# aiforvision/OCTA-autosegmentation

Hardware: AMD Instinct MI355X
Metric: synthetic OCTA samples/sec (graph + 304x304 image + 1216x1216 label triples) (higher is better)
Workload: dtype f64

## Files before the change

include/octa_hip.h:

```cpp
#ifndef OCTA_HIP_H
#define OCTA_HIP_H

#include <stddef.h>
#include <stdint.h>

#ifdef __cplusplus
extern "C" {
#endif

typedef struct octa_ctx octa_ctx;


int octa_abi_version(void);

const char *octa_last_error(void);

int octa_ctx_create(int device, octa_ctx **out);
void octa_ctx_destroy(octa_ctx *ctx);

size_t octa_ctx_scratch_bytes(const octa_ctx *ctx);

int octa_rasterize_2d(octa_ctx *ctx, int B, const double *d_edges, const int64_t *h_edge_off,
                      const uint8_t *d_keep, int no_pixels_x, int no_pixels_y, int mip_axis,
                      double min_radius, double max_radius, uint8_t *d_out, void *stream);
// ... 140 lines not shown
int octa_menten_floater(octa_ctx *ctx, const double *d_img, const int *d_pts, const int *d_npts, const int *d_dilations, const double *d_weights,
                        int radius, int B, int P, int N, unsigned char *d_mask, int *d_dist, double *d_tmp, double *d_out, void *stream);
int octa_menten_motion(octa_ctx *ctx, const void *d_in, void *d_out, int elem_size, const int *d_table, const void *d_white, int n_white,
                       int unit_elems, int B, int H, int W, void *stream);

int octa_noise_model(octa_ctx *ctx, const float *d_img, const float *d_background, const float *d_grids, int B, int H, int W, int gh, int gw,
                     uint64_t seed, uint32_t sample_offset, double lambda_delta, double lambda_speckle, double lambda_gamma,
                     const float *d_delta_in, const float *d_n_in, float *d_out, float *d_maps, float *d_fields, void *stream);
void octa_philox4x32_10(const uint32_t *counter4, const uint32_t *key2, uint32_t *out4);

int octa_noise_model_backward(octa_ctx *ctx, const float *d_dout, const float *d_img, const float *d_background, const float *d_grids, int B, int H,
                              int W, int gh, int gw, uint64_t seed, uint32_t sample_offset, double lambda_delta, double lambda_speckle,
                              double lambda_gamma, const float *d_delta_in, const float *d_n_in, float *d_dgrids, float *d_dmaps, float *d_out,
                              float *d_maps, float *d_logodds, float *d_bgrad, void *stream);

int octa_conv3x3_c1_fwd(octa_ctx *ctx, const void *d_x, const float *d_w, void *d_y, int N, int H, int W, int Cout, double *d_stat, int nslot,
                        void *stream);
int octa_conv3x3_c1_wgrad(octa_ctx *ctx, const void *d_x, const void *d_dy, float *d_dw, int N, int H, int W, int Cout, void *stream);

int octa_dice_bce_fwd(octa_ctx *ctx, const void *d_logits, int dtype, const float *d_y, int B, int64_t n, double *d_sums, void *stream);
int octa_dice_bce_finish(octa_ctx *ctx, const double *d_sums, int B, int64_t n, double smooth_nr, double smooth_dr, float *d_loss, void *stream);
int octa_dice_bce_bwd(octa_ctx *ctx, const void *d_logits, int dtype, const float *d_y, int B, int64_t n, const double *d_sums,
                      const float *d_grad_out, float smooth_nr, float smooth_dr, void *d_dlogits, void *stream);

int octa_thinconv_expand(octa_ctx *ctx, const void *d_s, const void *d_w, const void *d_bias, void *d_out, int N, int Hs, int Ws, int C, int K,
                         int pad, int flip, float slope, void *stream);
int octa_thinconv_squeeze(octa_ctx *ctx, const void *d_a, const void *d_w, const void *d_bias, void *d_out, int N, int Ha, int Wa, int C, int K,
                          int pad, int flip, void *stream);
long long octa_thinconv_wgrad_scratch_floats(int N, int Ha, int C, int K);
int octa_lrelu_bwd_bf16(octa_ctx *ctx, const void *d_y, const void *d_dy, void *d_out, int64_t n, float slope, void *stream);
int octa_thinconv_wgrad(octa_ctx *ctx, const void *d_a, const void *d_s, void *d_scratch, void *d_g, void *d_asum, int N, int Ha, int Wa, int Hs,
                        int Ws, int C, int K, int pad, int flip, void *stream);

int octa_reflect_pad_fwd(octa_ctx *ctx, const void *d_in, void *d_out, int dtype, int B, int H, int W, int C, int pad, void *stream);
int octa_reflect_pad_bwd(octa_ctx *ctx, const void *d_in, void *d_out, int dtype, int B, int H, int W, int C, int pad, void *stream);
int octa_blur_down_fwd(octa_ctx *ctx, const void *d_in, void *d_out, int dtype, int B, int H, int W, int C, void *stream);
int octa_blur_down_bwd(octa_ctx *ctx, const void *d_in, void *d_out, int dtype, int B, int H, int W, int C, void *stream);
int octa_blur_up_fwd(octa_ctx *ctx, const void *d_in, void *d_out, int dtype, int B, int H, int W, int C, void *stream);
int octa_blur_up_bwd(octa_ctx *ctx, const void *d_in, void *d_out, int dtype, int B, int H, int W, int C, void *stream);

int octa_remove_small_objects(octa_ctx *ctx, const uint8_t *d_in, int B, int H, int W, int min_size, int connectivity,
                              uint8_t on_value, uint8_t *d_out, void *stream);

int octa_skeletonize(octa_ctx *ctx, const uint8_t *d_in, int B, int H, int W, uint8_t *d_out, int *passes, void *stream);


size_t octa_fft2_c2c_f64_workspace_bytes(int b, int h, int w);

int octa_fft2_c2c_f64(const void *d_in, void *d_out, int b, int h, int w, int inverse, void *d_ws, void *stream);

size_t octa_oof_workspace_bytes(int b, int h, int w);

int octa_oof_2d(const float *d_in, double *d_out, int b, int h, int w, void *d_ws, void *stream);

int octa_oof_2d_response(const float *d_in, double *d_out, int b, int h, int w, void *d_ws, void *stream);


size_t octa_frangi_workspace_bytes(int b, int h, int w, int n_scales);

int octa_frangi_2d(const float *d_in, double *d_out, int b, int h, int w, int n_scales, const int *radii, const double *weights, float in_scale,
                   double beta, double gamma, int black_ridges, void *d_ws, void *stream);

int octa_frangi_hessian(const float *d_in, float *d_hrr, float *d_hrc, float *d_hcc, int b, int h, int w, int radius, const double *weights,
                        float in_scale, int black_ridges, void *d_ws, void *stream);

int octa_frangi_eigenvalues(const float *d_in, float *d_l1, float *d_l2, float *d_gamma, int b, int h, int w, int radius, const double *weights,
                            float in_scale, int black_ridges, void *d_ws, void *stream);

typedef struct octa_sim octa_sim;

typedef struct {
    double param_scale, d, r;
    double faz_radius_mean, faz_radius_std;
    double rotation_radius;
    double faz_center[2];
    double size[3];
    int n_trees;
    int walls[4];
    int n_modes;
    double modes[8][13];
    int forest_type;
    double nerve_center[2];
    double nerve_radius;
    const uint8_t *geometry;
    int geometry_shape[3];
    int n_source_walls;
    int source_walls[6];
} octa_sim_config;

#define OCTA_BIF_MAX_ATTS 256
typedef struct {
    int sample, n;
    double pos[3];
    double r, kappa, d;
    double atts[OCTA_BIF_MAX_ATTS * 3];
} octa_bif_request;

typedef void (*octa_bif_fn)(int n_req, const octa_bif_request *reqs, double *out6, void *user);

int octa_bif_native_init(const char *blas_path, int n_kappa, const double *kappas, const double *cs, const double *sn,
                         octa_bif_fn fallback, void *fallback_user);
void octa_bif_native(int n_req, const octa_bif_request *reqs, double *out6, void *user);
int octa_bif_native_counts(int64_t *h_out2);

int octa_sim_create(octa_ctx *ctx, const octa_sim_config *cfg, int B, octa_sim **out);
int octa_sim_create_ex(octa_ctx *ctx, const octa_sim_config *cfg, int B, int build, octa_sim **out);
void octa_sim_destroy(octa_sim *sim);

long long octa_sim_launch_count(void);
int octa_order_wait_launch(octa_ctx *ctx, long long ticket, int timeout_us, int settle_us, int *d_out3, void *stream);

int octa_sim_run(octa_sim *sim, const uint32_t *h_np_seeds, const uint64_t *h_py_seeds, octa_bif_fn bif, void *user,
                 void *stream);

int octa_sim_run_states(octa_sim *sim, const double *h_faz_radius, const double *h_stumps, const uint32_t *h_np_states,
                        const uint32_t *h_py_states, octa_bif_fn bif, void *user, void *stream);
int octa_sim_np_state(octa_sim *sim, int sample, uint32_t *h_state625);

int octa_sim_edge_offsets(octa_sim *sim, int64_t *h_edge_off, int64_t *h_n_art);

int octa_sim_export_edges(octa_sim *sim, double *h_edges);

int octa_sim_export_edges_device(octa_sim *sim, double *d_edges, void *stream);

int octa_sim_trace(octa_sim *sim, int32_t *h_trace);

int octa_sim_stats(octa_sim *sim, int64_t *h_stats);

int octa_sim_kd_paths(octa_sim *sim, int64_t *h_paths);

int octa_sim_assign_paths(octa_sim *sim, int64_t *h_paths);

int octa_sim_spans(octa_sim *sim, int64_t *h_spans);

int octa_sim_timing(octa_sim *sim, double *h_out8);

int octa_sim_service_stats(octa_sim *sim, double *h_out5);

int octa_sim_geometry(int num_cus, int *h_out4);

int octa_sim_is_large(const octa_sim *sim);

int octa_sim_fields(octa_sim *sim, int sample, double *h_oxy, int64_t cap_oxy, int64_t *n_oxy, double *h_co2,
                    int64_t cap_co2, int64_t *n_co2);

int octa_sim_kat_kd_order(octa_ctx *ctx, const double *h_pts, int64_t n, const uint8_t *h_need, int32_t *h_indices);

int octa_sim_kat_kd_order_signflag(octa_ctx *ctx, const double *h_pts, int64_t n, const uint8_t *h_need, int32_t need_bits, int32_t *h_indices);

int octa_sim_kat_sample(octa_ctx *ctx, const double *h_cand, int64_t n_cand, const double *h_npos, const double *h_nrad, int64_t n_art,
                        double *h_oxy, int64_t n_oxy, int64_t cap_oxy, double eps_n, double eps_k, double eps_s, const double *h_cst8,
                        int64_t *h_n_out);

#ifdef __cplusplus
}
#endif
#endif
```

octa_autosegmentation_amd/_native.py:

```python
import contextlib
import ctypes
import os
import random as _random
import threading

import numpy as np

HERE = os.path.dirname(os.path.abspath(__file__))
LIB_PATH = os.environ.get("OCTA_HIP_LIB") or os.path.join(HERE, "liboctahip.so")

_lib = None
_ctxs = {}
_lock = threading.Lock()

c_void_p, c_int, c_double, c_size_t = ctypes.c_void_p, ctypes.c_int, ctypes.c_double, ctypes.c_size_t


def _struct(name, ints, ptrs):
    fields = [("struct_size", ctypes.c_uint32)] + [(k, c_int) for k in ints.split()] + [("slope", ctypes.c_float)] + [(k, c_void_p) for k in ptrs.split()]
    return type(name, (ctypes.Structure,), {"_fields_": fields})


Conv3x3Args = _struct("Conv3x3Args", "N H W Cin Cout stride in_dilation tap_mask out_scale out_off_y out_off_x C1 CY1 nslot",
                      "d_x d_x2 d_w d_y d_y2 d_scale1 d_shift1 d_scale2 d_shift2 d_stat_partials d_stat_slots d_residual")
Conv3x3WgradArgs = _struct("Conv3x3WgradArgs", "N H W Cin Cout stride tap_mask C1 out_mode", "d_x d_x2 d_dy d_dw d_scale1 d_shift1 d_scale2 d_shift2")
WGRAD_TAP_MAJOR, WGRAD_PARAM_ADD, WGRAD_PARAM_SET = 0, 1, 2

SIGNATURES = {
    "octa_abi_version": (c_int, []),
    "octa_last_error": (ctypes.c_char_p, []),
    "octa_ctx_create": (c_int, [c_int, ctypes.POINTER(c_void_p)]),
    "octa_ctx_destroy": (None, [c_void_p]),
    "octa_ctx_scratch_bytes": (c_size_t, [c_void_p]),
    "octa_rasterize_2d": (c_int, [c_void_p, c_int, c_void_p, c_void_p, c_void_p, c_int, c_int, c_int, c_double,
                                  c_double, c_void_p, c_void_p]),
    "octa_rasterize_2d_plan": (c_int, [c_void_p, c_int, c_void_p, c_void_p, c_void_p, c_int, c_int, c_int, c_double, c_double, c_void_p]),
    "octa_rasterize_2d_draw": (c_int, [c_void_p, c_void_p, c_void_p]),
    "octa_raster_prof": (c_int, [c_void_p, c_void_p]),
    "octa_fs_dither": (c_int, [c_void_p, c_int, c_void_p, c_int, c_int, c_void_p, c_void_p]),
    "octa_voxel_padded_dims": (c_int, [c_void_p, c_void_p]),
    "octa_voxelize_3d": (c_int, [c_void_p, c_int, c_void_p, c_void_p, c_void_p, c_void_p, c_double, c_double, c_int, c_void_p, c_void_p]),
    "octa_edges_read_back": (c_int, [c_void_p, c_void_p, c_void_p, ctypes.c_int64, c_void_p, c_void_p]),
    "octa_max_u8": (c_int, [c_void_p, c_void_p, c_void_p, c_void_p, c_size_t, c_void_p]),
    "octa_bif_native_init": (c_int, [ctypes.c_char_p, c_int, c_void_p, c_void_p, c_void_p, c_void_p, c_void_p]),
    "octa_bif_native": (None, [c_int, c_void_p, c_void_p, c_void_p]),
    "octa_bif_native_counts": (c_int, [c_void_p]),
    "octa_instnorm_lrelu_fwd": (c_int, [c_void_p] * 7 + [c_int, c_int, ctypes.c_int64, c_int, ctypes.c_float, ctypes.c_float, c_void_p]),
    "octa_instnorm_lrelu_bwd": (c_int, [c_void_p] * 10 + [c_int, c_int, ctypes.c_int64, c_int, ctypes.c_float, c_void_p]),
    "octa_csv_bytes_bound": (ctypes.c_int64, [ctypes.c_int64]),
    "octa_csv_format_edges": (ctypes.c_int64, [c_void_p, ctypes.c_int64, c_void_p, ctypes.c_int64]),
    "octa_csv_write_file": (c_int, [ctypes.c_char_p, c_void_p, ctypes.c_int64]),
    "octa_csv_count_rows": (ctypes.c_int64, [c_void_p, ctypes.c_int64]),
    "octa_csv_parse_edges": (ctypes.c_int64, [c_void_p, ctypes.c_int64, c_void_p, ctypes.c_int64]),
    "octa_py_random_advance": (c_int, [c_void_p, ctypes.c_int64]),
    "octa_png_write_gray8": (c_int, [ctypes.c_char_p, c_void_p, c_int, c_int, c_int]),
    "octa_png_write_bits": (c_int, [ctypes.c_char_p, c_void_p, c_int, c_int, c_int]),
    "octa_write_sample_files": (c_int, [ctypes.c_int64, c_void_p, c_void_p, c_void_p, c_void_p, c_void_p, c_int, c_int, c_void_p, c_int, c_int, c_int,
                                        ctypes.c_char_p, ctypes.c_int64, c_int, c_int]),
    "octa_pack_bits": (c_int, [c_void_p, c_void_p, c_void_p, ctypes.c_int64, c_int, c_void_p]),
    "octa_background_noise": (c_int, [c_void_p, c_void_p, c_void_p, c_void_p, ctypes.c_int64, c_void_p, c_void_p, c_void_p]),
    "octa_speckle_brightness": (c_int, [c_void_p, c_void_p, c_void_p, c_void_p, c_int, c_int, c_int, c_void_p, c_void_p, c_void_p]),
    "octa_menten_vessel_noise": (c_int, [c_void_p, c_void_p, c_int, c_void_p, c_void_p, c_void_p, c_int, c_double, c_double, c_int, c_int, c_int, c_void_p, c_void_p, c_void_p]),
    "octa_menten_floater_mask": (c_int, [c_void_p, c_void_p, c_void_p, c_void_p, c_int, c_int, c_int, c_void_p, c_void_p, c_void_p]),
    "octa_menten_floater": (c_int, [c_void_p, c_void_p, c_void_p, c_void_p, c_void_p, c_void_p, c_int, c_int, c_int, c_int, c_void_p, c_void_p, c_void_p, c_void_p, c_void_p]),
    "octa_menten_motion": (c_int, [c_void_p, c_void_p, c_void_p, c_int, c_void_p, c_void_p, c_int, c_int, c_int, c_int, c_int, c_void_p]),
    "octa_noise_model": (c_int, [c_void_p, c_void_p, c_void_p, c_void_p, c_int, c_int, c_int, c_int, c_int, ctypes.c_uint64, ctypes.c_uint32, c_double, c_double, c_double,
                                 c_void_p, c_void_p, c_void_p, c_void_p, c_void_p, c_void_p]),
    "octa_noise_model_backward": (c_int, [c_void_p, c_void_p, c_void_p, c_void_p, c_void_p, c_int, c_int, c_int, c_int, c_int, ctypes.c_uint64, ctypes.c_uint32,
                                          c_double, c_double, c_double, c_void_p, c_void_p, c_void_p, c_void_p, c_void_p, c_void_p, c_void_p, c_void_p, c_void_p]),
    "octa_philox4x32_10": (None, [c_void_p, c_void_p, c_void_p]),
    "octa_sim_create": (c_int, [c_void_p, c_void_p, c_int, ctypes.POINTER(c_void_p)]),
    "octa_sim_create_ex": (c_int, [c_void_p, c_void_p, c_int, c_int, ctypes.POINTER(c_void_p)]),
    "octa_sim_destroy": (None, [c_void_p]),
    "octa_sim_run": (c_int, [c_void_p, c_void_p, c_void_p, c_void_p, c_void_p, c_void_p]),
    "octa_sim_run_states": (c_int, [c_void_p, c_void_p, c_void_p, c_void_p, c_void_p, c_void_p, c_void_p, c_void_p]),
    "octa_sim_np_state": (c_int, [c_void_p, c_int, c_void_p]),
    "octa_thinconv_expand": (c_int, [c_void_p, c_void_p, c_void_p, c_void_p, c_void_p, c_int, c_int, c_int, c_int, c_int, c_int, c_int, ctypes.c_float, c_void_p]),
    "octa_thinconv_squeeze": (c_int, [c_void_p, c_void_p, c_void_p, c_void_p, c_void_p, c_int, c_int, c_int, c_int, c_int, c_int, c_int, c_void_p]),
    "octa_lrelu_bwd_bf16": (c_int, [c_void_p, c_void_p, c_void_p, c_void_p, ctypes.c_int64, ctypes.c_float, c_void_p]),
    "octa_thinconv_wgrad_scratch_floats": (ctypes.c_longlong, [c_int, c_int, c_int, c_int]),
    "octa_thinconv_wgrad": (c_int, [c_void_p, c_void_p, c_void_p, c_void_p, c_void_p, c_void_p, c_int, c_int, c_int, c_int, c_int, c_int, c_int, c_int, c_int, c_void_p]),
    "octa_sim_spans": (c_int, [c_void_p, c_void_p]),
    "octa_sim_edge_offsets": (c_int, [c_void_p, c_void_p, c_void_p]),
    "octa_sim_export_edges": (c_int, [c_void_p, c_void_p]),
    "octa_sim_export_edges_device": (c_int, [c_void_p, c_void_p, c_void_p]),
    "octa_sim_trace": (c_int, [c_void_p, c_void_p]),
    "octa_sim_stats": (c_int, [c_void_p, c_void_p]),
    "octa_sim_kd_paths": (c_int, [c_void_p, c_void_p]),
    "octa_sim_assign_paths": (c_int, [c_void_p, c_void_p]),
    "octa_sim_timing": (c_int, [c_void_p, c_void_p]),
    "octa_sim_service_stats": (c_int, [c_void_p, c_void_p]),
    "octa_sim_geometry": (c_int, [c_int, c_void_p]),
    "octa_sim_is_large": (c_int, [c_void_p]),
    "octa_conv2d_f32_nchw": (c_int, [c_void_p, c_void_p, c_void_p, c_void_p, c_void_p] + [c_int] * 14 + [c_void_p]),
    "octa_convtranspose2x2_f32_nchw": (c_int, [c_void_p, c_void_p, c_void_p, c_void_p, c_int, c_int, c_int, c_int, c_int, c_void_p]),
    "octa_conv2d_f32_dgrad_nchw": (c_int, [c_void_p, c_void_p, c_void_p, c_void_p] + [c_int] * 11 + [c_void_p]),
    "octa_conv2d_f32_wgrad_workspace": (c_int, [c_int] * 10 + [ctypes.POINTER(c_size_t)]),
    "octa_conv2d_f32_wgrad_nchw": (c_int, [c_void_p, c_void_p, c_void_p, c_void_p, c_void_p, c_void_p, c_size_t] + [c_int] * 10 + [c_void_p]),
    "octa_sim_fields": (c_int, [c_void_p, c_int, c_void_p, ctypes.c_int64, c_void_p, c_void_p, ctypes.c_int64, c_void_p]),
    "octa_instnorm_lrelu_nhwc_bwd": (c_int, [c_void_p, c_void_p, c_void_p, c_void_p, c_void_p, c_void_p, c_void_p, c_void_p, c_void_p, c_void_p, c_int, c_int, ctypes.c_int64, ctypes.c_float, c_void_p]),
    "octa_pack_conv_weights": (c_int, [c_void_p, c_void_p, c_int, c_void_p, c_void_p]),
    "octa_head1_nhwc_bwd": (c_int, [c_void_p, c_void_p, c_void_p, c_void_p, ctypes.c_int64, c_int, c_void_p, c_void_p, c_void_p, c_void_p]),
    "octa_instnorm_nhwc_stats": (c_int, [c_void_p, c_void_p, c_void_p, c_void_p, c_void_p, c_void_p, c_void_p, c_void_p, c_int, c_int, ctypes.c_int64, ctypes.c_float, c_void_p]),
    "octa_scale_shift_lrelu_nhwc": (c_int, [c_void_p, c_void_p, c_void_p, c_void_p, c_void_p, c_int, c_int, ctypes.c_int64, ctypes.c_float, c_void_p]),
    "octa_resize_bilinear": (c_int, [c_void_p, c_void_p, c_int, c_int, c_int, c_int, c_void_p, c_int, c_int, c_void_p, c_void_p, c_void_p]),
    "octa_resize_bilinear_bwd": (c_int, [c_void_p, c_void_p, c_int, c_int, c_int, c_int, c_int, c_void_p, c_void_p]),
    "octa_flip_rot90_rotate": (c_int, [c_void_p, c_void_p, c_void_p, c_int, c_int, c_void_p, c_void_p, c_void_p, ctypes.c_float, c_int, c_void_p]),
    "octa_remove_small_objects": (c_int, [c_void_p, c_void_p, c_int, c_int, c_int, c_int, c_int, ctypes.c_uint8, c_void_p, c_void_p]),
    "octa_skeletonize": (c_int, [c_void_p, c_void_p, c_int, c_int, c_int, c_void_p, ctypes.POINTER(c_int), c_void_p]),
    "octa_reflect_pad_fwd": (c_int, [c_void_p, c_void_p, c_void_p, c_int, c_int, c_int, c_int, c_int, c_int, c_void_p]),
    "octa_reflect_pad_bwd": (c_int, [c_void_p, c_void_p, c_void_p, c_int, c_int, c_int, c_int, c_int, c_int, c_void_p]),
    "octa_blur_down_fwd": (c_int, [c_void_p, c_void_p, c_void_p, c_int, c_int, c_int, c_int, c_int, c_void_p]),
    "octa_blur_down_bwd": (c_int, [c_void_p, c_void_p, c_void_p, c_int, c_int, c_int, c_int, c_int, c_void_p]),
    "octa_blur_up_fwd": (c_int, [c_void_p, c_void_p, c_void_p, c_int, c_int, c_int, c_int, c_int, c_void_p]),
    "octa_blur_up_bwd": (c_int, [c_void_p, c_void_p, c_void_p, c_int, c_int, c_int, c_int, c_int, c_void_p]),
    "octa_conv4x4_nhwc_fwd": (c_int, [c_void_p, c_void_p, c_void_p, c_void_p, c_int, c_int, c_int, c_int, c_int, c_int, c_void_p]),
    "octa_conv4x4_nhwc_wgrad": (c_int, [c_void_p, c_void_p, c_void_p, c_void_p, c_int, c_int, c_int, c_int, c_int, c_void_p]),
    "octa_dice_bce_fwd": (c_int, [c_void_p, c_void_p, c_int, c_void_p, c_int, ctypes.c_int64, c_void_p, c_void_p]),
    "octa_dice_bce_finish": (c_int, [c_void_p, c_void_p, c_int, ctypes.c_int64, c_double, c_double, c_void_p, c_void_p]),
    "octa_dice_bce_bwd": (c_int, [c_void_p, c_void_p, c_int, c_void_p, c_int, ctypes.c_int64, c_void_p, c_void_p, ctypes.c_float, ctypes.c_float, c_void_p, c_void_p]),
    "octa_sim_launch_count": (ctypes.c_longlong, []),
    "octa_order_wait_launch": (c_int, [c_void_p, ctypes.c_longlong, c_int, c_int, c_void_p, c_void_p]),
    "octa_conv3x3_c1_wgrad": (c_int, [c_void_p, c_void_p, c_void_p, c_void_p, c_int, c_int, c_int, c_int, c_void_p]),
    "octa_conv_stat_tiles": (c_int, [c_int, c_int]),
    "octa_instnorm_lrelu_head1_nhwc_bwd": (c_int, [c_void_p, c_void_p, c_void_p, c_void_p, c_void_p, c_void_p, c_void_p, c_void_p, c_void_p, c_void_p, c_void_p, c_void_p, c_void_p, c_int, c_int, ctypes.c_int64, ctypes.c_float, c_void_p]),
    "octa_conv3x3_s2t_nhwc": (c_int, [c_void_p, c_void_p, c_void_p, c_void_p, c_int, c_int, c_int, c_int, c_int, c_int, c_void_p, c_void_p]),
    "octa_conv3x3_nhwc_fwd": (c_int, [c_void_p, ctypes.POINTER(Conv3x3Args), c_void_p]),
    "octa_conv3x3_nhwc_wgrad": (c_int, [c_void_p, ctypes.POINTER(Conv3x3WgradArgs), c_void_p]),
    "octa_conv3x3_nhwc_fwd_pad": (c_int, [c_void_p, c_void_p, c_void_p, c_void_p, c_int, c_int, c_int, c_int, c_int, c_int, c_int, c_void_p, c_int, c_void_p]),
    "octa_conv3x3_nhwc_wgrad_pad": (c_int, [c_void_p, c_void_p, c_void_p, c_void_p, c_int, c_int, c_int, c_int, c_int, c_int, c_int, c_int, c_void_p]),
    "octa_instnorm_lrelu_nhwc_fwd": (c_int, [c_void_p] * 7 + [c_int, c_int, ctypes.c_int64, ctypes.c_float, ctypes.c_float, c_void_p, c_int, c_void_p, c_int, c_void_p]),
    "octa_instnorm_lrelu_head1_nhwc_fwd": (c_int, [c_void_p] * 9 + [c_int, c_int, ctypes.c_int64, ctypes.c_float, ctypes.c_float, c_void_p, c_int, c_void_p]),
    "octa_head1_nhwc_fwd": (c_int, [c_void_p, c_void_p, c_void_p, c_void_p, ctypes.c_int64, c_int, c_void_p, c_void_p]),
    "octa_headn_nhwc_fwd": (c_int, [c_void_p, c_void_p, c_void_p, c_void_p, c_int, ctypes.c_int64, c_int, c_int, c_void_p, c_void_p]),
    "octa_headn_nhwc_bwd": (c_int, [c_void_p, c_void_p, c_void_p, c_void_p, c_int, ctypes.c_int64, c_int, c_int, c_void_p, c_void_p, c_void_p, c_void_p]),
    "octa_conv3x3_c1_fwd": (c_int, [c_void_p, c_void_p, c_void_p, c_void_p, c_int, c_int, c_int, c_int, c_void_p, c_int, c_void_p]),
    "octa_fft2_c2c_f64_workspace_bytes": (c_size_t, [c_int, c_int, c_int]),
    "octa_fft2_c2c_f64": (c_int, [c_void_p, c_void_p, c_int, c_int, c_int, c_int, c_void_p, c_void_p]),
    "octa_oof_workspace_bytes": (c_size_t, [c_int, c_int, c_int]),
    "octa_oof_2d": (c_int, [c_void_p, c_void_p, c_int, c_int, c_int, c_void_p, c_void_p]),
    "octa_oof_2d_response": (c_int, [c_void_p, c_void_p, c_int, c_int, c_int, c_void_p, c_void_p]),
    "octa_frangi_workspace_bytes": (c_size_t, [c_int, c_int, c_int, c_int]),
    "octa_frangi_2d": (c_int, [c_void_p, c_void_p, c_int, c_int, c_int, c_int, c_void_p, c_void_p, ctypes.c_float, c_double, c_double, c_int, c_void_p, c_void_p]),
    "octa_frangi_hessian": (c_int, [c_void_p, c_void_p, c_void_p, c_void_p, c_int, c_int, c_int, c_int, c_void_p, ctypes.c_float, c_int, c_void_p, c_void_p]),
    "octa_frangi_eigenvalues": (c_int, [c_void_p, c_void_p, c_void_p, c_void_p, c_int, c_int, c_int, c_int, c_void_p, ctypes.c_float, c_int, c_void_p, c_void_p]),
    "octa_sim_kat_kd_order": (c_int, [c_void_p, c_void_p, ctypes.c_int64, c_void_p, c_void_p]),
    "octa_sim_kat_kd_order_signflag": (c_int, [c_void_p, c_void_p, ctypes.c_int64, c_void_p, ctypes.c_int32, c_void_p]),
    "octa_sim_kat_sample": (c_int, [c_void_p, c_void_p, ctypes.c_int64, c_void_p, c_void_p, ctypes.c_int64, c_void_p, ctypes.c_int64, ctypes.c_int64,
                                    c_double, c_double, c_double, c_void_p, c_void_p]),
}


class OctaHipError(RuntimeError):
    pass


def lib():
    global _lib
    if _lib is None:
        with _lock:
            if _lib is None:
                if not os.path.exists(LIB_PATH):
                    raise OctaHipError(
                        f"{LIB_PATH} is missing: build it with `python -m octa_autosegmentation_amd.build` "
                        "(hipcc --offload-arch=gfx950). There is no CPU fallback.")
                import torch
                l = ctypes.CDLL(LIB_PATH)
                for name, (res, args) in SIGNATURES.items():
                    fn = getattr(l, name)
                    fn.restype = res
                    fn.argtypes = args
                _lib = l
    return _lib


_SYNC_DEBUG = bool(os.environ.get("OCTA_SYNC_DEBUG"))


def check(rc, what):
    if _SYNC_DEBUG and rc == 0:
        import sys
        import torch
        torch.cuda.current_stream().synchronize()
        print(f"[octa-sync] {threading.current_thread().name} {what} ok", file=sys.stderr, flush=True)
    if rc != 0:
        msg = lib().octa_last_error().decode("utf-8", "replace")
        raise OctaHipError(f"{what} failed (rc={rc}): {msg}")


_tls = threading.local()


def _device_index(device_index):
    import torch
    if not torch.cuda.is_available():
        raise OctaHipError("no ROCm GPU visible to torch; the HIP path cannot run (no CPU fallback)")
    return int(torch.cuda.current_device() if device_index is None else device_index)


def _create_ctx(device_index):
    out = c_void_p()
    call("octa_ctx_create", device_index, ctypes.byref(out))
    return out


def new_ctx(device_index=None):
    return _create_ctx(_device_index(device_index))


def free_ctx(h):
    if h is not None:
        lib().octa_ctx_destroy(h)


@contextlib.contextmanager
def use_ctx(h):
    prev = getattr(_tls, "ctx", None)
    _tls.ctx = h
    try:
        yield h
    finally:
        _tls.ctx = prev


def ctx(device_index=None):
    import torch
    if getattr(_tls, "ctx", None) is not None:
        return _tls.ctx
    device_index = _device_index(device_index)
    key = (device_index, threading.get_ident(), torch.cuda.current_stream(device_index).cuda_stream)
    with _lock:
        h = _ctxs.get(key)
    if h is None:
        h = _create_ctx(device_index)
        with _lock:
            _ctxs[key] = h
    return h


def current_stream_ptr():
    import torch
    return c_void_p(torch.cuda.current_stream().cuda_stream)


def addr(t):
    return t.data_ptr() if t is not None else None


def _ctx_of(device):
    return ctx(device.index)



def launch(name, device, *args, what=None, ctx=None, stream=None):
    argv = [_ctx_of(device) if ctx is None else ctx]
    for a in args:
        argv.append(a.data_ptr() if hasattr(a, "data_ptr") else a)
    argv.append(current_stream_ptr() if stream is None else stream)
    check(getattr(lib(), name)(*argv), what or name)


def call(name, *args, what=None):
    check(getattr(lib(), name)(*[a.data_ptr() if hasattr(a, "data_ptr") else a for a in args]), what or name)


def advance_python_random(n):
    if n <= 0:
        return
    if n < 64:
        for _ in range(n):
            _random.random()
        return
    ver, state, gauss = _random.getstate()
    arr = np.array(state, dtype=np.uint32)
    call("octa_py_random_advance", arr.ctypes.data, int(n))
    _random.setstate((ver, tuple(arr.tolist()), gauss))
```

octa_autosegmentation_amd/csrc/sim.hip:

```cpp

#include <chrono>
#include <vector>

#include "common.h"
#include "sim_host.h"
#include <thread>
#include <atomic>
#include <cstdlib>
#include <cstring>

using namespace OCTA_SIMK;

#if OCTA_SIM_LARGE
#define OCTA_SIM_T octa_simL_impl
#define OCTA_SIM_FN(name) octa_simL_##name
#else
#define OCTA_SIM_T octa_simS_impl
#define OCTA_SIM_FN(name) octa_simS_##name
#endif
#define octa_sim_create OCTA_SIM_FN(create)
#define octa_sim_destroy OCTA_SIM_FN(destroy)
#define octa_sim_run OCTA_SIM_FN(run)
#define octa_sim_run_states OCTA_SIM_FN(run_states)
#define octa_sim_np_state OCTA_SIM_FN(np_state)
#define octa_sim_edge_offsets OCTA_SIM_FN(edge_offsets)
#define octa_sim_export_edges OCTA_SIM_FN(export_edges)
#define octa_sim_export_edges_device OCTA_SIM_FN(export_edges_device)
#define octa_sim_trace OCTA_SIM_FN(trace)
#define octa_sim_stats OCTA_SIM_FN(stats)
#define octa_sim_kd_paths OCTA_SIM_FN(kd_paths)
#define octa_sim_assign_paths OCTA_SIM_FN(assign_paths)
#define octa_sim_fields OCTA_SIM_FN(fields)
#define octa_sim_service_stats OCTA_SIM_FN(service_stats)
#define octa_sim_geometry OCTA_SIM_FN(geometry)
#define octa_sim_spans OCTA_SIM_FN(spans)
#define octa_sim_timing OCTA_SIM_FN(timing)
#define octa_sim_kat_kd_order OCTA_SIM_FN(kat_kd_order)
#define octa_sim_kat_kd_order_signflag OCTA_SIM_FN(kat_kd_order_signflag)
#define octa_sim_kat_sample OCTA_SIM_FN(kat_sample)
struct OCTA_SIM_T;
extern "C" void octa_sim_destroy(OCTA_SIM_T *S);
extern "C" long long octa_sim_next_ticket(void);
extern "C" int *octa_sim_launch_flag(int device);

namespace {

constexpr int SIM_THREADS = SIM_THREADS_PER_WG;
constexpr int SIM_WG_PER_CU = 2;
#if OCTA_SIM_LARGE
constexpr size_t SIM_LDS = 2048;
#else
constexpr size_t SIM_LDS = SIM_LDS_BYTES;
static_assert((size_t)KD_MAILBOX_OFF + KD_MAILBOX_BYTES <= (size_t)SIM_USER_BYTES && SIM_WG_PER_CU * SIM_LDS <= 160 * 1024, "LDS budget");
#endif
static_assert((624 + 1248) * 4 <= SEQ_SIDE_LDS, "the Mersenne-Twister state and queue of the candidate stream fit the side-job LDS");
static_assert(SIM_THREADS == 64 * KD_WAVES, "kd mailboxes are sized for KD_WAVES waves");
constexpr int REQ_CAP = 8192;

static_assert(sizeof(BifRequest) == sizeof(octa_bif_request), "request layout must match the public header");
static_assert(MAXKEPT == OCTA_BIF_MAX_ATTS, "request capacity must match the public header");

struct BatchPtrs {
    double *npos[2], *nrad[2], *nkap[2];
    int *npar[2], *nch0[2], *nch1[2];
    unsigned char *nnch[2], *nact[2];
    double *oxy, *co2, *cand, *py_u;
    unsigned *py_state;
    int *nn, *act_list;
    int *nn_prev[2];
    double *nn_d2[2];
    unsigned *sorted;
    int *gnode, *gstart, *gcount;
    Rec *rec;
    int *glist, *child_group;
    FlushRec *fl_rec;
    idx_t *kd_idx, *kd_rank;
    unsigned char *removed, *ven_near;
    unsigned long long *hashes;
    unsigned *pairs;
    unsigned long long *set_hash;
    int *set_key, *tmp_int;
    double *grid_pts;
    unsigned *cand_idx;
    double *tmp_dbl;
    SampleScalars *sc;
    IterParams *iters;
    BifRequest *reqs;
    int *req_count;
    double *bif_results;
    unsigned *mt_state;
    unsigned short *valid;
    size_t valid_stride;
    unsigned *valid_count;
    int *n_per_iter;
    int *next_sample;
    unsigned char *wg_scratch;
#ifdef OCTA_SIM_DEBUG_SAT
    int *dbg;
#endif
    int *trace;
    int n_samples;
    SimConst C;
};

__device__ __forceinline__ SimArrays sample_arrays(const BatchPtrs &B, int s) {
    SimArrays A;
    for (int f = 0; f < 2; f++) {
        A.npos[f] = B.npos[f] + (size_t)s * NCAP * 3;
        A.nrad[f] = B.nrad[f] + (size_t)s * NCAP;
        A.nkap[f] = B.nkap[f] + (size_t)s * NCAP;
        A.npar[f] = B.npar[f] + (size_t)s * NCAP;
        A.nch0[f] = B.nch0[f] + (size_t)s * NCAP;
        A.nch1[f] = B.nch1[f] + (size_t)s * NCAP;
        A.nnch[f] = B.nnch[f] + (size_t)s * NCAP;
        A.nact[f] = B.nact[f] + (size_t)s * NCAP;
        A.nn_prev[f] = B.nn_prev[f] + (size_t)s * OCAP;
        A.nn_d2[f] = B.nn_d2[f] + (size_t)s * OCAP;
    }
    A.oxy = B.oxy + (size_t)s * OCAP * 3;
    A.co2 = B.co2 + (size_t)s * CCAP * 3;
    A.cand = B.cand + (size_t)s * NCANDCAP * 3;
    A.py_u = B.py_u + (size_t)s * PYCAP;
    A.nn = B.nn + (size_t)s * OCAP;
    A.act_list = B.act_list + (size_t)s * NCAP;
    A.sorted = B.sorted + (size_t)s * SORTCAP;
    A.gnode = B.gnode + (size_t)s * GCAP;
    A.gstart = B.gstart + (size_t)s * GCAP;
    A.gcount = B.gcount + (size_t)s * GCAP;
    A.rec = B.rec + (size_t)s * GCAP;
    A.glist = B.glist + (size_t)s * GCAP;
    A.child_group = B.child_group + (size_t)s * NCAP;
    A.fl_rec = B.fl_rec + (size_t)s * 2 * MURRAY_FLUSH_LDS;
    A.kd_idx = B.kd_idx + (size_t)s * OCAP;
    A.kd_rank = B.kd_rank + (size_t)s * OCAP;
    A.removed = B.removed + (size_t)s * OCAP;
    A.ven_near = B.ven_near + (size_t)s * OCAP;
    A.hashes = B.hashes + (size_t)s * OCAP;
    A.pairs = B.pairs + (size_t)s * PCAP;
    A.set_hash = B.set_hash + (size_t)s * SETCAP;
    A.set_key = B.set_key + (size_t)s * SETCAP;
    A.tmp_int = B.tmp_int + (size_t)s * (OCAP + 2 * NCANDCAP);
    A.grid_pts = B.grid_pts + (size_t)s * GRID_N * 3;
    A.tmp_dbl = B.tmp_dbl + (size_t)s * OCAP * 3;
    A.sc = B.sc + s;
#ifdef OCTA_SIM_DEBUG_SAT
    A.dbg = B.dbg ? B.dbg + (size_t)s * B.C.n_iter * 16 : nullptr;
    A.dbg_it = 0;
#endif
    return A;
}

struct WaveMt {
    unsigned *st;
    unsigned *ob;
    int cur, avail;
    int lane;
    __device__ void regen_block() {
        for (int c = 0; c < 623; c += 64) {
            int k = c + lane;
            unsigned nv = 0;
            if (k < 623) {
                unsigned y = (st[k] & 0x80000000u) | (st[k + 1] & 0x7fffffffu);
                unsigned m = (k < 227) ? st[k + 397] : st[k - 227];
                nv = m ^ (y >> 1) ^ ((y & 1u) ? 0x9908b0dfu : 0u);
            }
            __builtin_amdgcn_wave_barrier();
            if (k < 623) st[k] = nv;
            __builtin_amdgcn_wave_barrier();
        }
        if (lane == 0) {
            unsigned y = (st[623] & 0x80000000u) | (st[0] & 0x7fffffffu);
            st[623] = st[396] ^ (y >> 1) ^ ((y & 1u) ? 0x9908b0dfu : 0u);
        }
        __builtin_amdgcn_wave_barrier();
    }
    __device__ static unsigned temper(unsigned y) {
        y ^= (y >> 11);
        y ^= (y << 7) & 0x9d2c5680u;
        y ^= (y << 15) & 0xefc60000u;
        y ^= (y >> 18);
        return y;
    }
    __device__ void ensure(int k) {
        if (avail - cur >= k) return;
        const int rem = avail - cur;
        for (int c = 0; c < rem; c += 64) {
            int i = c + lane;
            unsigned v = (i < rem) ? ob[cur + i] : 0u;
            __builtin_amdgcn_wave_barrier();
            if (i < rem) ob[i] = v;
            __builtin_amdgcn_wave_barrier();
        }
// ... 1030 lines not shown
            return hipMemcpy2DAsync(dst, n * elem, src, cap_elems * elem, n * elem, (size_t)B, hipMemcpyDeviceToHost, stream);
        };
        OCTA_HIP_CHECK(get(pos[f], P.npos[f], 24, NCAP)); OCTA_HIP_CHECK(get(rad[f], P.nrad[f], 8, NCAP));
        OCTA_HIP_CHECK(get(par[f], P.npar[f], 4, NCAP)); OCTA_HIP_CHECK(get(c0[f], P.nch0[f], 4, NCAP));
        OCTA_HIP_CHECK(get(c1[f], P.nch1[f], 4, NCAP)); OCTA_HIP_CHECK(get(nch[f], P.nnch[f], 1, NCAP));
    }
    OCTA_HIP_CHECK(hipStreamSynchronize(stream));
    long total = 0;
    for (int s = 0; s < B; s++) {
        const SampleScalars &sc = S->h_sc[s];
        const double *cp[2], *cr[2];
        const int *cpar[2], *cc0[2], *cc1[2];
        const unsigned char *cn[2];
        for (int f = 0; f < 2; f++) {
            const size_t n = (size_t)nmax[f];
            cp[f] = pos[f] + (size_t)s * n * 3; cr[f] = rad[f] + (size_t)s * n; cpar[f] = par[f] + (size_t)s * n;
            cc0[f] = c0[f] + (size_t)s * n; cc1[f] = c1[f] + (size_t)s * n; cn[f] = nch[f] + (size_t)s * n;
        }
        long n_art = 0;
        long ne = export_edges(cp, cr, cpar, cc0, cc1, cn, sc.n_nodes, S->cfg.n_trees, h_edges + 7 * total, 1L << 40, &n_art);
        if (ne < 0) { octa::set_error("octa_sim_export_edges: export failed"); return -1; }
        total += ne;
    }
    return 0;
}

extern "C" int octa_sim_export_edges_device(OCTA_SIM_T *S, double *d_edges, void *stream_) {
    if (!S || !S->ran || !d_edges) { octa::set_error("octa_sim_export_edges_device: run the simulation first"); return -2; }
    OCTA_HIP_CHECK(hipSetDevice(S->ctx->device));
    hipStream_t stream = (hipStream_t)stream_;
    const int B = S->B;
    std::vector<long> off(B + 1, 0);
    for (int s = 0; s < B; s++) off[s + 1] = off[s] + (S->h_sc[s].n_nodes[0] - S->cfg.n_trees) + (S->h_sc[s].n_nodes[1] - S->cfg.n_trees);
    if (!S->d_edge_off) OCTA_HIP_CHECK(hipMalloc(&S->d_edge_off, sizeof(long) * (B + 1)));
    OCTA_HIP_CHECK(hipMemcpyAsync(S->d_edge_off, off.data(), sizeof(long) * (B + 1), hipMemcpyHostToDevice, stream));
    OCTA_HIP_CHECK(hipStreamSynchronize(stream));
    const size_t lds = OCTA_SIM_LARGE ? 2048 : 2048 + (size_t)NCAP * 2 * sizeof(idx_t);
    hipLaunchKernelGGL(sim_export_kernel, dim3((unsigned)B, 2), dim3(256), lds, stream, S->P, S->d_edge_off, S->cfg.n_trees, d_edges);
    OCTA_HIP_CHECK(hipGetLastError());
    return 0;
}

extern "C" int octa_sim_trace(OCTA_SIM_T *S, int32_t *h_trace) {
    if (!S || !S->ran || !h_trace) { octa::set_error("octa_sim_trace: run the simulation first"); return -2; }
    OCTA_HIP_CHECK(hipSetDevice(S->ctx->device));
    OCTA_HIP_CHECK(hipMemcpy(h_trace, S->P.trace, sizeof(int32_t) * (size_t)S->B * S->iters.size() * 4, hipMemcpyDeviceToHost));
    return 0;
}

extern "C" int octa_sim_stats(OCTA_SIM_T *S, int64_t *h_stats) {
    if (!S || !S->ran || !h_stats) { octa::set_error("octa_sim_stats: run the simulation first"); return -2; }
    for (int s = 0; s < S->B; s++) {
        const SampleScalars &sc = S->h_sc[s];
        int64_t *o = h_stats + 32 * s;
        o[0] = sc.err; o[1] = sc.py_pos; o[2] = sc.murray_steps; o[3] = sc.n_bif; o[4] = sc.respec;
        o[5] = sc.n_nodes[0]; o[6] = sc.n_nodes[1];
        memcpy(&o[7], &sc.faz_radius, 8);
        for (int k = 0; k < 16; k++) o[8 + k] = sc.prof[k];
        for (int k = 0; k < 8; k++) o[24 + k] = sc.kdprof[k];
    }
    return 0;
}

extern "C" int octa_sim_kd_paths(OCTA_SIM_T *S, int64_t *h_paths) {
    if (!S || !S->ran || !h_paths) { octa::set_error("octa_sim_kd_paths: run the simulation first"); return -2; }
    for (int s = 0; s < S->B; s++)
        for (int k = 0; k < 3; k++) h_paths[3 * s + k] = S->h_sc[s].kd_path[k];
    return 0;
}

extern "C" int octa_sim_assign_paths(OCTA_SIM_T *S, int64_t *h_paths) {
    if (!S || !S->ran || !h_paths) { octa::set_error("octa_sim_assign_paths: run the simulation first"); return -2; }
    for (int s = 0; s < S->B; s++) { h_paths[2 * s] = S->h_sc[s].assign_path[0]; h_paths[2 * s + 1] = S->h_sc[s].assign_path[1]; }
    return 0;
}

extern "C" int octa_sim_fields(OCTA_SIM_T *S, int sample, double *h_oxy, int64_t cap_oxy, int64_t *n_oxy, double *h_co2,
                               int64_t cap_co2, int64_t *n_co2) {
    if (!S || !S->ran || sample < 0 || sample >= S->B) { octa::set_error("octa_sim_fields: bad arguments"); return -2; }
    OCTA_HIP_CHECK(hipSetDevice(S->ctx->device));
    const SampleScalars &sc = S->h_sc[sample];
    if (n_oxy) *n_oxy = sc.n_oxy;
    if (n_co2) *n_co2 = sc.n_co2;
    if (h_oxy) {
        int64_t n = sc.n_oxy < cap_oxy ? sc.n_oxy : cap_oxy;
        OCTA_HIP_CHECK(hipMemcpy(h_oxy, S->P.oxy + (size_t)sample * OCAP * 3, sizeof(double) * 3 * n, hipMemcpyDeviceToHost));
    }
    if (h_co2) {
        int64_t n = sc.n_co2 < cap_co2 ? sc.n_co2 : cap_co2;
        OCTA_HIP_CHECK(hipMemcpy(h_co2, S->P.co2 + (size_t)sample * CCAP * 3, sizeof(double) * 3 * n, hipMemcpyDeviceToHost));
    }
    return 0;
}

#if !OCTA_SIM_LARGE
namespace {
__global__ void __launch_bounds__(SIM_THREADS)
sim_kat_kd_kernel(const double *pts, int n, const unsigned char *need, idx_t *out_idx, idx_t *out_rank, float *xy, double zlo, double zhi,
                  int flag_in_sign, int need_bits) {
    extern __shared__ __attribute__((aligned(16))) unsigned char smem[];
    Blk b = {(int)threadIdx.x, (int)blockDim.x, smem};
    kd_build(b, pts, n, out_idx, out_rank, xy, zlo, zhi, nullptr, need, flag_in_sign != 0, (unsigned char)need_bits);
}

int kat_kd_order(octa_ctx *ctx, const double *h_pts, int64_t n, const uint8_t *h_need, int32_t *h_indices, int flag_in_sign, int need_bits);
}

extern "C" int octa_sim_kat_kd_order(octa_ctx *ctx, const double *h_pts, int64_t n, const uint8_t *h_need, int32_t *h_indices) {
    if (!ctx || !h_pts || !h_indices || n < 0 || n > OCAP) { octa::set_error("octa_sim_kat_kd_order: bad arguments"); return -2; }
    return kat_kd_order(ctx, h_pts, n, h_need, h_indices, 0, 0xff);
}

extern "C" int octa_sim_kat_kd_order_signflag(octa_ctx *ctx, const double *h_pts, int64_t n, const uint8_t *h_need, int32_t need_bits, int32_t *h_indices) {
    if (!ctx || !h_pts || !h_need || !h_indices || n < 0 || n > OCAP || need_bits <= 0 || need_bits > 0xff) { octa::set_error("octa_sim_kat_kd_order_signflag: bad arguments"); return -2; }
    for (int64_t i = 0; i < n; i++)
        if (!(h_pts[3 * i] >= 0.0)) { octa::set_error("octa_sim_kat_kd_order_signflag: x must be >= 0"); return -2; }
    return kat_kd_order(ctx, h_pts, n, h_need, h_indices, 1, need_bits);
}

namespace {
int kat_kd_order(octa_ctx *ctx, const double *h_pts, int64_t n, const uint8_t *h_need, int32_t *h_indices, int flag_in_sign, int need_bits) {
    if (n == 0) return 0;
    OCTA_HIP_CHECK(hipSetDevice(ctx->device));
    double *d_pts = nullptr;
    unsigned char *d_need = nullptr;
    idx_t *d_idx = nullptr;
    float *d_xy = nullptr;
    double zlo = h_pts[2], zhi = h_pts[2];
    for (int64_t i = 1; i < n; i++) { zlo = h_pts[3 * i + 2] < zlo ? h_pts[3 * i + 2] : zlo; zhi = h_pts[3 * i + 2] > zhi ? h_pts[3 * i + 2] : zhi; }
    OCTA_HIP_CHECK(hipMalloc(&d_xy, sizeof(float) * 2 * n));
    OCTA_HIP_CHECK(hipMalloc(&d_pts, sizeof(double) * 3 * n));
    OCTA_HIP_CHECK(hipMalloc(&d_idx, sizeof(idx_t) * 2 * n));
    OCTA_HIP_CHECK(hipMemcpy(d_pts, h_pts, sizeof(double) * 3 * n, hipMemcpyHostToDevice));
    if (h_need) {
        OCTA_HIP_CHECK(hipMalloc(&d_need, n));
        OCTA_HIP_CHECK(hipMemcpy(d_need, h_need, n, hipMemcpyHostToDevice));
    }
    OCTA_HIP_CHECK(hipFuncSetAttribute(reinterpret_cast<const void *>(sim_kat_kd_kernel), hipFuncAttributeMaxDynamicSharedMemorySize, (int)SIM_LDS));
    hipLaunchKernelGGL(sim_kat_kd_kernel, dim3(1), dim3(SIM_THREADS), SIM_LDS, 0, d_pts, (int)n, d_need, d_idx, d_idx + n, d_xy, zlo, zhi, flag_in_sign, need_bits);
    OCTA_HIP_CHECK(hipGetLastError());
    std::vector<idx_t> h(n);
    OCTA_HIP_CHECK(hipMemcpy(h.data(), d_idx, sizeof(idx_t) * n, hipMemcpyDeviceToHost));
    for (int64_t i = 0; i < n; i++) h_indices[i] = (int32_t)h[i];
    (void)hipFree(d_pts); (void)hipFree(d_idx); (void)hipFree(d_xy); if (d_need) (void)hipFree(d_need);
    return 0;
}

__global__ void __launch_bounds__(SIM_THREADS)
sim_kat_sample_kernel(SimArrays A, SimConst C, IterParams P) {
    extern __shared__ __attribute__((aligned(16))) unsigned char smem[];
    Blk b = {(int)threadIdx.x, (int)blockDim.x, smem};
    phase_sample(b, A, C, P, 0);
}
}

extern "C" int octa_sim_kat_sample(octa_ctx *ctx, const double *h_cand, int64_t n_cand, const double *h_npos, const double *h_nrad, int64_t n_art,
                                   double *h_oxy, int64_t n_oxy, int64_t cap_oxy, double eps_n, double eps_k, double eps_s, const double *h_cst8,
                                   int64_t *h_n_out) {
    if (!ctx || !h_cst8 || !h_n_out || n_cand < 0 || n_cand > NCANDCAP || n_art < 0 || n_art > NCAP || n_oxy < 0 || n_oxy > OCAP || cap_oxy < n_oxy ||
        (n_cand && !h_cand) || (n_art && (!h_npos || !h_nrad)) || (cap_oxy && !h_oxy)) {
        octa::set_error("octa_sim_kat_sample: bad arguments");
        return -2;
    }
    OCTA_HIP_CHECK(hipSetDevice(ctx->device));
    SimConst C;
    memset(&C, 0, sizeof(C));
    C.ps = h_cst8[0]; C.sx = h_cst8[1]; C.sy = h_cst8[2]; C.sz = h_cst8[3]; C.gs = h_cst8[4]; C.fc0 = h_cst8[5]; C.fc1 = h_cst8[6];
    SampleScalars sc;
    memset(&sc, 0, sizeof(sc));
    sc.faz_radius = h_cst8[7]; sc.n_nodes[0] = (int)n_art; sc.n_oxy = (int)n_oxy;
    IterParams P;
    memset(&P, 0, sizeof(P));
    P.N = (int)n_cand; P.eps_n = eps_n; P.eps_k = eps_k; P.eps_s = eps_s;
    const size_t n_dbl = (size_t)OCAP * 3 * 2 + (size_t)GRID_N * 3 + (size_t)NCANDCAP * 3 + (size_t)NCAP * 4;
    const size_t n_int = (size_t)OCAP + 2 * (size_t)NCANDCAP, n_byte = (size_t)(OCAP > NCANDCAP ? OCAP : NCANDCAP);
    const size_t off_int = n_dbl * 8, off_byte = off_int + n_int * 4, off_sc = (off_byte + n_byte + 15) & ~(size_t)15;
    unsigned char *d = nullptr;
    OCTA_HIP_CHECK(hipMalloc(&d, off_sc + sizeof(SampleScalars)));
    int rc = 0;
    auto ok = [&](hipError_t e, const char *what) { if (e != hipSuccess && rc == 0) { octa::set_error("octa_sim_kat_sample: %s: %s", what, hipGetErrorString(e)); rc = -1; } return rc == 0; };
    double *dd = reinterpret_cast<double *>(d);
    SimArrays A;
    memset((void *)&A, 0, sizeof(A));
    A.oxy = dd; A.tmp_dbl = dd + (size_t)OCAP * 3; A.grid_pts = A.tmp_dbl + (size_t)OCAP * 3;
    double *d_cand = A.grid_pts + (size_t)GRID_N * 3;
    A.cand = d_cand; A.npos[0] = d_cand + (size_t)NCANDCAP * 3; A.nrad[0] = A.npos[0] + (size_t)NCAP * 3;
    A.tmp_int = reinterpret_cast<int *>(d + off_int); A.removed = d + off_byte; A.sc = reinterpret_cast<SampleScalars *>(d + off_sc);
    if (ok(hipMemset(d, 0, off_sc), "clear") && (!n_cand || ok(hipMemcpy(d_cand, h_cand, sizeof(double) * 3 * n_cand, hipMemcpyHostToDevice), "candidates")) &&
        (!n_art || (ok(hipMemcpy(A.npos[0], h_npos, sizeof(double) * 3 * n_art, hipMemcpyHostToDevice), "nodes") &&
                    ok(hipMemcpy(A.nrad[0], h_nrad, sizeof(double) * n_art, hipMemcpyHostToDevice), "radii"))) &&
        (!n_oxy || ok(hipMemcpy(A.oxy, h_oxy, sizeof(double) * 3 * n_oxy, hipMemcpyHostToDevice), "sinks")) &&
        ok(hipMemcpy(A.sc, &sc, sizeof(sc), hipMemcpyHostToDevice), "scalars") &&
        ok(hipFuncSetAttribute(reinterpret_cast<const void *>(sim_kat_sample_kernel), hipFuncAttributeMaxDynamicSharedMemorySize, (int)SIM_LDS), "attribute")) {
        hipLaunchKernelGGL(sim_kat_sample_kernel, dim3(1), dim3(SIM_THREADS), SIM_LDS, 0, A, C, P);
        if (ok(hipGetLastError(), "launch") && ok(hipMemcpy(&sc, A.sc, sizeof(sc), hipMemcpyDeviceToHost), "result")) {
            if (sc.err) { octa::set_error("octa_sim_kat_sample: the phase set error bits %d", sc.err); rc = -3; }
            else {
                *h_n_out = sc.n_oxy;
                const int64_t n = sc.n_oxy < cap_oxy ? sc.n_oxy : cap_oxy;
                if (n) ok(hipMemcpy(h_oxy, A.oxy, sizeof(double) * 3 * n, hipMemcpyDeviceToHost), "sinks back");
            }
        }
    }
    (void)hipFree(d);
    return rc;
}

#endif

extern "C" int octa_sim_service_stats(OCTA_SIM_T *S, double *h_out4) {
    if (!S || !S->ran || !h_out4) { octa::set_error("octa_sim_service_stats: run the simulation first"); return -2; }
    h_out4[0] = (double)S->diag_tickets; h_out4[1] = S->diag_max_gap_ms; h_out4[2] = (double)S->diag_relaunches; h_out4[3] = (double)S->diag_parked;
    h_out4[4] = S->diag_max_bif_ms;
    return 0;
}

extern "C" int octa_sim_geometry(int num_cus, int *h_out4) {
    if (!h_out4) { octa::set_error("octa_sim_geometry: null output"); return -2; }
    h_out4[0] = SIM_THREADS; h_out4[1] = SIM_WG_PER_CU; h_out4[2] = (int)SIM_LDS; h_out4[3] = SIM_WG_PER_CU * (num_cus > 0 ? num_cus : 256);
    return 0;
}

extern "C" int octa_sim_spans(OCTA_SIM_T *S, int64_t *h_spans) {
    if (!S || !S->ran || !h_spans) { octa::set_error("octa_sim_spans: run the simulation first"); return -2; }
    for (int s = 0; s < S->B; s++) { h_spans[2 * s] = S->h_sc[s].t_begin; h_spans[2 * s + 1] = S->h_sc[s].t_end; }
    return 0;
}

extern "C" int octa_sim_timing(OCTA_SIM_T *S, double *h_out8) {
    if (!S || !S->ran || !h_out8) { octa::set_error("octa_sim_timing: run the simulation first"); return -2; }
    h_out8[0] = S->ms_a; h_out8[1] = (double)S->n_a; h_out8[2] = S->ms_b; h_out8[3] = (double)S->n_b;
    h_out8[4] = S->ms_total; h_out8[5] = S->ms_host_bif; h_out8[6] = (double)S->n_bif_req; h_out8[7] = (double)S->bytes;
    return 0;
}
```

octa_autosegmentation_amd/csrc/sim_api.cpp:

```cpp
#include <cstdlib>
#include <cstring>
#include <new>

#include "common.h"

extern "C" {
struct octa_simS_impl;
struct octa_simL_impl;
#define OCTA_DECL(SFX, T)                                                                                                                       \
    int octa_sim##SFX##_create(octa_ctx *, const octa_sim_config *, int, T **);                                                                 \
    void octa_sim##SFX##_destroy(T *);                                                                                                          \
    int octa_sim##SFX##_run(T *, const uint32_t *, const uint64_t *, octa_bif_fn, void *, void *);                                              \
    int octa_sim##SFX##_run_states(T *, const double *, const double *, const uint32_t *, const uint32_t *, octa_bif_fn, void *, void *);       \
    int octa_sim##SFX##_np_state(T *, int, uint32_t *);                                                                                         \
    int octa_sim##SFX##_edge_offsets(T *, int64_t *, int64_t *);                                                                                \
    int octa_sim##SFX##_export_edges(T *, double *);                                                                                            \
    int octa_sim##SFX##_export_edges_device(T *, double *, void *);                                                                             \
    int octa_sim##SFX##_trace(T *, int32_t *);                                                                                                  \
    int octa_sim##SFX##_stats(T *, int64_t *);                                                                                                  \
    int octa_sim##SFX##_kd_paths(T *, int64_t *);                                                                                               \
    int octa_sim##SFX##_assign_paths(T *, int64_t *);                                                                                           \
    int octa_sim##SFX##_spans(T *, int64_t *);                                                                                                  \
    int octa_sim##SFX##_timing(T *, double *);                                                                                                  \
    int octa_sim##SFX##_service_stats(T *, double *);                                                                                           \
    int octa_sim##SFX##_geometry(int, int *);                                                                                                   \
    int octa_sim##SFX##_fields(T *, int, double *, int64_t, int64_t *, double *, int64_t, int64_t *);
OCTA_DECL(S, octa_simS_impl)
OCTA_DECL(L, octa_simL_impl)
#undef OCTA_DECL
int octa_simS_kat_kd_order(octa_ctx *, const double *, int64_t, const uint8_t *, int32_t *);
int octa_simS_kat_kd_order_signflag(octa_ctx *, const double *, int64_t, const uint8_t *, int32_t, int32_t *);
int octa_simS_kat_sample(octa_ctx *, const double *, int64_t, const double *, const double *, int64_t, double *, int64_t, int64_t, double, double, double,
                         const double *, int64_t *);
}

#include <atomic>
#include <mutex>
static std::atomic<long long> g_sim_launches{0};
extern "C" long long octa_sim_next_ticket(void) { return g_sim_launches.fetch_add(1, std::memory_order_acq_rel) + 1; }
extern "C" long long octa_sim_launch_count(void) { return g_sim_launches.load(std::memory_order_acquire); }
extern "C" int *octa_sim_launch_flag(int device) {
    static std::mutex m;
    static int *flags[64] = {};
    if (device < 0 || device >= 64) return nullptr;
    std::lock_guard<std::mutex> g(m);
    if (!flags[device]) {
        int prev = 0;
        if (hipGetDevice(&prev) != hipSuccess || hipSetDevice(device) != hipSuccess) return nullptr;
        int *p = nullptr;
        if (hipMalloc(&p, 64) != hipSuccess || hipMemset(p, 0, 64) != hipSuccess || hipDeviceSynchronize() != hipSuccess) { (void)hipSetDevice(prev); return nullptr; }
        (void)hipSetDevice(prev);
        flags[device] = p;
    }
    return flags[device];
}

struct octa_sim {
    bool large = false;
    octa_simS_impl *s = nullptr;
    octa_simL_impl *l = nullptr;
};

static bool wants_large(const octa_sim_config *c) {
    if (const char *e = getenv("OCTA_SIM_BUILD")) {
        if (!strcmp(e, "large")) return true;
        if (!strcmp(e, "default")) return false;
    }
    if (c->param_scale <= 6.0) return false;
    int iters = 0, nmax = 0;
    for (int m = 0; m < c->n_modes && m < 8; m++) {
        const int I = (int)c->modes[m][0], N = (int)c->modes[m][1];
        if (I > 0) { iters += I; nmax = N > nmax ? N : nmax; }
    }
    return nmax > 8192 / 3 && iters > 40;
}

#define FWD(call_s, call_l) (sim->large ? (call_l) : (call_s))

extern "C" int octa_sim_create_ex(octa_ctx *ctx, const octa_sim_config *cfg, int B, int build, octa_sim **out) {
    if (!out || !cfg || build < 0 || build > 2) { octa::set_error("octa_sim_create: bad arguments"); return -2; }
    *out = nullptr;
    octa_sim *sim = new (std::nothrow) octa_sim();
    if (!sim) { octa::set_error("octa_sim_create: out of host memory"); return -1; }
    sim->large = build == 0 ? wants_large(cfg) : build == 2;
    const int rc = sim->large ? octa_simL_create(ctx, cfg, B, &sim->l) : octa_simS_create(ctx, cfg, B, &sim->s);
    if (rc) { delete sim; return rc; }
    *out = sim;
    return 0;
}
extern "C" int octa_sim_create(octa_ctx *ctx, const octa_sim_config *cfg, int B, octa_sim **out) { return octa_sim_create_ex(ctx, cfg, B, 0, out); }
extern "C" void octa_sim_destroy(octa_sim *sim) {
    if (!sim) return;
    if (sim->large) octa_simL_destroy(sim->l); else octa_simS_destroy(sim->s);
    delete sim;
}
#define NEED(sim, what) if (!(sim)) { octa::set_error(what ": null simulator"); return -2; }
extern "C" int octa_sim_run(octa_sim *sim, const uint32_t *a, const uint64_t *b, octa_bif_fn f, void *u, void *st) {
    NEED(sim, "octa_sim_run") return FWD(octa_simS_run(sim->s, a, b, f, u, st), octa_simL_run(sim->l, a, b, f, u, st));
}
extern "C" int octa_sim_run_states(octa_sim *sim, const double *fz, const double *stp, const uint32_t *a, const uint32_t *b, octa_bif_fn f, void *u, void *st) {
    NEED(sim, "octa_sim_run_states") return FWD(octa_simS_run_states(sim->s, fz, stp, a, b, f, u, st), octa_simL_run_states(sim->l, fz, stp, a, b, f, u, st));
}
extern "C" int octa_sim_np_state(octa_sim *sim, int k, uint32_t *o) { NEED(sim, "octa_sim_np_state") return FWD(octa_simS_np_state(sim->s, k, o), octa_simL_np_state(sim->l, k, o)); }
extern "C" int octa_sim_edge_offsets(octa_sim *sim, int64_t *a, int64_t *b) { NEED(sim, "octa_sim_edge_offsets") return FWD(octa_simS_edge_offsets(sim->s, a, b), octa_simL_edge_offsets(sim->l, a, b)); }
extern "C" int octa_sim_export_edges(octa_sim *sim, double *e) { NEED(sim, "octa_sim_export_edges") return FWD(octa_simS_export_edges(sim->s, e), octa_simL_export_edges(sim->l, e)); }
extern "C" int octa_sim_export_edges_device(octa_sim *sim, double *e, void *st) {
    NEED(sim, "octa_sim_export_edges_device") return FWD(octa_simS_export_edges_device(sim->s, e, st), octa_simL_export_edges_device(sim->l, e, st));
}
extern "C" int octa_sim_trace(octa_sim *sim, int32_t *t) { NEED(sim, "octa_sim_trace") return FWD(octa_simS_trace(sim->s, t), octa_simL_trace(sim->l, t)); }
extern "C" int octa_sim_stats(octa_sim *sim, int64_t *t) { NEED(sim, "octa_sim_stats") return FWD(octa_simS_stats(sim->s, t), octa_simL_stats(sim->l, t)); }
extern "C" int octa_sim_kd_paths(octa_sim *sim, int64_t *t) { NEED(sim, "octa_sim_kd_paths") return FWD(octa_simS_kd_paths(sim->s, t), octa_simL_kd_paths(sim->l, t)); }
extern "C" int octa_sim_assign_paths(octa_sim *sim, int64_t *t) { NEED(sim, "octa_sim_assign_paths") return FWD(octa_simS_assign_paths(sim->s, t), octa_simL_assign_paths(sim->l, t)); }
extern "C" int octa_sim_spans(octa_sim *sim, int64_t *t) { NEED(sim, "octa_sim_spans") return FWD(octa_simS_spans(sim->s, t), octa_simL_spans(sim->l, t)); }
extern "C" int octa_sim_timing(octa_sim *sim, double *t) { NEED(sim, "octa_sim_timing") return FWD(octa_simS_timing(sim->s, t), octa_simL_timing(sim->l, t)); }
extern "C" int octa_sim_service_stats(octa_sim *sim, double *t) { NEED(sim, "octa_sim_service_stats") return FWD(octa_simS_service_stats(sim->s, t), octa_simL_service_stats(sim->l, t)); }
extern "C" int octa_sim_fields(octa_sim *sim, int k, double *o, int64_t co, int64_t *no, double *c, int64_t cc, int64_t *nc) {
    NEED(sim, "octa_sim_fields") return FWD(octa_simS_fields(sim->s, k, o, co, no, c, cc, nc), octa_simL_fields(sim->l, k, o, co, no, c, cc, nc));
}
extern "C" int octa_sim_geometry(int num_cus, int *h_out4) { return octa_simS_geometry(num_cus, h_out4); }
extern "C" int octa_sim_kat_kd_order(octa_ctx *ctx, const double *p, int64_t n, const uint8_t *need, int32_t *o) { return octa_simS_kat_kd_order(ctx, p, n, need, o); }
extern "C" int octa_sim_kat_kd_order_signflag(octa_ctx *ctx, const double *p, int64_t n, const uint8_t *need, int32_t bits, int32_t *o) { return octa_simS_kat_kd_order_signflag(ctx, p, n, need, bits, o); }
extern "C" int octa_sim_kat_sample(octa_ctx *ctx, const double *cand, int64_t n_cand, const double *npos, const double *nrad, int64_t n_art, double *oxy,
                                   int64_t n_oxy, int64_t cap_oxy, double eps_n, double eps_k, double eps_s, const double *cst8, int64_t *n_out) {
    return octa_simS_kat_sample(ctx, cand, n_cand, npos, nrad, n_art, oxy, n_oxy, cap_oxy, eps_n, eps_k, eps_s, cst8, n_out);
}
extern "C" int octa_sim_is_large(const octa_sim *sim) { return sim && sim->large ? 1 : 0; }
```

octa_autosegmentation_amd/csrc/sim_core.h:

```cpp
#pragma once
#include <cmath>
#include <cstdint>
#include <cstring>
#include <algorithm>
#include "gpow.h"
#include "glibc_trig.h"

#ifndef OCTA_SIM_LARGE
#define OCTA_SIM_LARGE 0
#endif
#if OCTA_SIM_LARGE
#define OCTA_SIMK octa_simk_large
#else
#define OCTA_SIMK octa_simk
#endif
namespace OCTA_SIMK {

#if OCTA_SIM_LARGE
typedef unsigned int idx_t;
typedef unsigned long long kdw_t;
constexpr int IDX_BITS = 18;
constexpr int GROUP_BITS = 17;
constexpr int NCAP = 1 << 17;
constexpr int OCAP = 1 << 18;
// ... 781 lines not shown
            inc += __builtin_amdgcn_update_dpp(0, inc, 0x114, 0xf, 0xf, true);
            inc += __builtin_amdgcn_update_dpp(0, inc, 0x118, 0xf, 0xf, true);
            totS = __shfl(inc, TW - 1, TW);
        }
        const int preS = inc - nS;
        const int cut = base + totS;
        {
            int g = (p0 - base) - preS;
#pragma unroll
            for (int w = 0; w < NW; w++) {
                const int q0 = p0 + 64 * w;
                int lim = ((p1 < cut) ? p1 : cut) - q0;
                if (lim <= 0) continue;
                unsigned long long inv = ~ms[w];
                if (lim < 64) inv &= (1ull << lim) - 1ull;
                while (inv) {
                    int i = (int)__ffsll((long long)inv) - 1;
                    inv &= inv - 1ull;
                    box[g++] = (idx_t)(q0 + i);
                }
            }
        }
        __builtin_amdgcn_wave_barrier();
        {
            int r = totS - preS - nS;
#pragma unroll
            for (int w = NW - 1; w >= 0; w--) {
                const int q0 = p0 + 64 * w;
                if (q0 >= p1) continue;
                unsigned long long sm = ms[w];
                if (cut > q0) { int sh = cut - q0; sm = (sh >= 64) ? 0ull : (sm >> sh) << sh; }
                while (sm) {
                    int i = 63 - __clzll((long long)sm);
                    sm &= ~(1ull << i);
                    kd_swap(a, q0 + i, (int)box[r++]);
                }
            }
        }
        __builtin_amdgcn_wave_barrier();
        if (cut <= nth) first = cut; else last = cut;
    }
    if (tl == 0) kd_insertion_sort(a, first, last);
    __builtin_amdgcn_wave_barrier();
}
constexpr int KD_MASK_MAX = 16000;
__device__ inline void kd_nth_element_wave_long(const KdPair &a, int first, int nth, int last, idx_t *mb) {
    const int tl = (int)(threadIdx.x & 63);
    if (first == last || nth == last) return;
    idx_t *box = mb + ((first + 1) >> 1);
    int n = last - first, lg = 0;
    while ((n >> (lg + 1)) > 0) lg++;
    int depth = lg * 2;
    while (last - first > KD_MASK_MAX) {
        if (depth == 0) {
            if (tl == 0) { kd_heap_select(a, first, nth + 1, last); kd_swap(a, first, nth); }
            __builtin_amdgcn_wave_barrier();
            return;
        }
        --depth;
        if (tl == 0) kd_median_to_first(a, first, last);
        __builtin_amdgcn_wave_barrier();
        const kdw_t pk = a.kv[first];
        const int base = first + 1, m = last - base;
        const int c = ((m + 63) / 64) | 1;
        int p0 = base + tl * c;
        if (p0 > last) p0 = last;
        const int p1 = (p0 + c < last) ? p0 + c : last;
        int nS = 0;
        for (int i = p0; i < p1; i++) nS += kd_less_w(a, a.kv[i], pk) ? 1 : 0;
        int inc = nS;
#pragma unroll
        for (int d = 1; d < 64; d <<= 1) {
            int u = __shfl_up(inc, d, 64);
            if (tl >= d) inc += u;
        }
        const int totS = __shfl(inc, 63, 64);
        const int preS = inc - nS;
        const int cut = base + totS;
        {
            int g = (p0 - base) - preS;
            const int lim = p1 < cut ? p1 : cut;
            for (int i = p0; i < lim; i++)
                if (!kd_less_w(a, a.kv[i], pk)) box[g++] = (idx_t)i;
        }
        __builtin_amdgcn_wave_barrier();
        {
            int r = totS - preS - nS;
            const int lo = p0 > cut ? p0 : cut;
            for (int i = p1 - 1; i >= lo; i--)
                if (kd_less_w(a, a.kv[i], pk)) kd_swap(a, i, (int)box[r++]);
        }
        __builtin_amdgcn_wave_barrier();
        if (cut <= nth) first = cut; else last = cut;
    }
    kd_nth_element_team<64, 4>(a, first, nth, last, true, mb, depth);
}
#endif

OCTA_HD inline unsigned f32_bits(float v) { unsigned u; memcpy(&u, &v, 4); return u; }
OCTA_HD inline unsigned f32_sortable(float v) {
    unsigned u;
    memcpy(&u, &v, 4);
    return (u >> 31) ? ~u : (u | 0x80000000u);
}
OCTA_HD inline float f32_unsortable(unsigned e) {
    unsigned u = (e >> 31) ? (e & 0x7fffffffu) : ~e;
    float v;
    memcpy(&v, &u, 4);
    return v;
}
OCTA_HD inline float f32_round_up(double x) {
#if defined(__HIP_DEVICE_COMPILE__)
    return __double2float_ru(x);
#else
    float f = (float)x;
    return (double)f < x ? nextafterf(f, INFINITY) : f;
#endif
}
OCTA_HD inline float f32_round_down(double x) {
#if defined(__HIP_DEVICE_COMPILE__)
    return __double2float_rd(x);
#else
    float f = (float)x;
    return (double)f > x ? nextafterf(f, -INFINITY) : f;
#endif
}
OCTA_HD inline double f32_ulp(float v) {
    const float a = fabsf(v);
    return (double)nextafterf(a, INFINITY) - (double)a;
}
OCTA_HD inline void atomic_max_u32(unsigned *p, unsigned v) {
#if defined(__HIP_DEVICE_COMPILE__)
    atomicMax(p, v);
#else
    if (v > *p) *p = v;
#endif
}
OCTA_HD inline void atomic_min_u32(unsigned *p, unsigned v) {
#if defined(__HIP_DEVICE_COMPILE__)
    atomicMin(p, v);
#else
    if (v < *p) *p = v;
#endif
}

constexpr int KD_TAB_OFF = OCAP * (int)sizeof(kdw_t);
constexpr int KD_BOX_BYTES = KD_RANGES * 24;
static_assert(KD_RANGES >= OCAP / 17 + 1, "ranges per level");
static_assert(KD_MAILBOX_OFF % 16 == 0 && KD_MAILBOX_OFF >= KD_TAB_OFF + KD_RANGES * KD_TAB_BYTES_PER_RANGE, "kd tables overlap the mailbox");
static_assert(KD_MAILBOX_OFF + (KD_BOX_BYTES > KD_MAILBOX_BYTES ? KD_BOX_BYTES : KD_MAILBOX_BYTES) <= SIM_USER_BYTES, "kd table layout (box table and mailbox share their area)");
OCTA_HD inline void kd_build(const Blk &b, const double *pts, int n, idx_t *out_idx, idx_t *out_rank,
                              float *xy, double zlo, double zhi, long *kdprof = nullptr, const unsigned char *need = nullptr,
                              const bool flag_in_sign = false, const unsigned char need_bits = 0xff) {
#if defined(__HIP_DEVICE_COMPILE__) && !defined(OCTA_SIM_PROF_ASSIGN) && !defined(OCTA_SIM_PROF_SAMPLE) && !defined(OCTA_SIM_PROF_SET) && !defined(OCTA_SIM_PROF_MAIL) && !defined(OCTA_SIM_PROF_SEQ) && !defined(OCTA_SIM_PROF_SEQ2)
#define KDP(slot) do { if (kdprof && b.tid == 0) { long _t = (long)wall_clock64(); kdprof[slot] += _t - _kt; _kt = _t; } } while (0)
    long _kt = (long)wall_clock64();
#else
#define KDP(slot) do { } while (0)
#endif
    kdw_t *kv = reinterpret_cast<kdw_t *>(b.user_of<1>());
    idx_t *tab = reinterpret_cast<idx_t *>(b.user_of<1>() + KD_TAB_OFF);
    idx_t *rs = tab, *re = tab + KD_RANGES;
    idx_t *rs2 = tab + 2 * KD_RANGES, *re2 = tab + 3 * KD_RANGES;
    signed char *rd = reinterpret_cast<signed char *>(tab + 4 * KD_RANGES);
    unsigned *bbf = reinterpret_cast<unsigned *>(b.user_of<1>() + KD_MAILBOX_OFF);
#if defined(__HIP_DEVICE_COMPILE__) && !OCTA_SIM_LARGE
    if ((size_t)n * (sizeof(kdw_t) + 8) + 8 <= (size_t)KD_TAB_OFF)
        xy = reinterpret_cast<float *>(b.user_of<1>() + (((size_t)n * sizeof(kdw_t) + 7) & ~(size_t)7));
#endif
    for (int i = b.tid; i < n; i += b.nth) {
        kv[i] = (kdw_t)i;
        const float fx = (float)pts[3 * i];
        xy[2 * i] = (flag_in_sign && (need[i] & need_bits)) ? -fx : fx; xy[2 * i + 1] = (float)pts[3 * i + 1];
    }
    int *live_n = b.coll() + KD_COLL_LIVE_N;
    if (b.tid == 0) { rs[0] = 0; re[0] = (idx_t)n; *live_n = n; }
    const float z_up = f32_round_up(zhi), z_dn = f32_round_down(zlo);
    b.sync();
    int nr = (n > 16) ? 1 : 0;
    while (nr > 0) {
        for (int q = b.tid; q < nr; q += b.nth) {
            for (int k = 0; k < 2; k++) { bbf[6 * q + k] = 0u; bbf[6 * q + 3 + k] = ~0u; }
            bbf[6 * q + 2] = f32_sortable(z_up); bbf[6 * q + 5] = f32_sortable(z_dn);
            rd[q] = 0;
        }
        b.sync();
        const int live = OCTA_UNI(*live_n);
        const bool sparse = live <= KD_SPARSE_MAX && 2 * live <= n && nr <= KD_SPARSE_RANGES;
        const int span = sparse ? live : n;
        {
            const int chunk = ((span + b.nth - 1) / b.nth) | 1;
            const int i0 = b.tid * chunk, i1 = (i0 + chunk < span) ? i0 + chunk : span;
            int q = 0, vs = 0, ve = 0;
            if (i0 < i1 && !sparse) {
                int lo_ = 0, hi_ = nr - 1;
                while (lo_ < hi_) { int mid = (lo_ + hi_ + 1) >> 1; if (rs[mid] <= i0) lo_ = mid; else hi_ = mid - 1; }
                q = lo_;
            }
            if (i0 < i1 && sparse) {
                ve = (int)re[0] - (int)rs[0];
                while (i0 >= ve && q + 1 < nr) { q++; vs = ve; ve = vs + (int)re[q] - (int)rs[q]; }
            }
            bool have = false, hit = false;
            float mx[2] = {0, 0}, mn[2] = {0, 0};
            auto flush = [&](int qq) {
                for (int k = 0; k < 2; k++) {
                    atomic_max_u32(&bbf[6 * qq + k], f32_sortable(nextafterf(mx[k], INFINITY)));
                    atomic_min_u32(&bbf[6 * qq + 3 + k], f32_sortable(nextafterf(mn[k], -INFINITY)));
                }
            };
            constexpr int KB = 8;
            int qw = q, cs = 0, ce = 0, ns = 0x7fffffff;
            if (i0 < i1) { cs = rs[qw]; ce = re[qw]; ns = qw + 1 < nr ? (int)rs[qw + 1] : 0x7fffffff; }
            for (int ib = i0; ib < i1; ib += KB) {
                int eq[KB], eid[KB];
                kdw_t ew[KB];
                if (sparse) {
#pragma unroll
                    for (int k = 0; k < KB; k++) {
                        const int i = ib + k;
                        eq[k] = -1; eid[k] = 0;
                        if (i < i1) {
                            while (i >= ve && qw + 1 < nr) { qw++; cs = rs[qw]; ce = re[qw]; vs = ve; ve = vs + ce - cs; }
                            const int at = cs + (i - vs);
                            if (at < ce) { eq[k] = qw; eid[k] = at; }
                        }
                    }
#pragma unroll
                    for (int k = 0; k < KB; k++) eid[k] = (int)(kv[eid[k]] & KD_IDX_MASK);
                } else {
#pragma unroll
                    for (int k = 0; k < KB; k++) ew[k] = kv[ib + k < i1 ? ib + k : i1 - 1];
#pragma unroll
                    for (int k = 0; k < KB; k++) {
                        const int i = ib + k;
                        eq[k] = -1; eid[k] = 0;
                        if (i < i1) {
                            while (i >= ns) { qw++; cs = ns; ce = re[qw]; ns = qw + 1 < nr ? (int)rs[qw + 1] : 0x7fffffff; }
                            if (i >= cs && i < ce) { eq[k] = qw; eid[k] = (int)(ew[k] & KD_IDX_MASK); }
                        }
                    }
                }
                float ex[KB], ey[KB];
                unsigned char nd[KB];
#pragma unroll
                for (int k = 0; k < KB; k++) {
                    const float sx = xy[2 * eid[k]];
                    ex[k] = flag_in_sign ? fabsf(sx) : sx; ey[k] = xy[2 * eid[k] + 1];
                    nd[k] = flag_in_sign ? (unsigned char)(f32_bits(sx) >> 31) : (need ? (unsigned char)(need[eid[k]] & need_bits) : (unsigned char)1);
                }
#pragma unroll
                for (int k = 0; k < KB; k++) {
                    if (eq[k] < 0) continue;
                    if (eq[k] != q) {
                        if (have) { flush(q); have = false; }
                        if (hit) { rd[q] = 1; hit = false; }
                        q = eq[k];
                    }
                    if (nd[k]) hit = true;
                    if (!have) { mx[0] = mn[0] = ex[k]; mx[1] = mn[1] = ey[k]; }
                    else {
                        mx[0] = mx[0] > ex[k] ? mx[0] : ex[k]; mn[0] = mn[0] < ex[k] ? mn[0] : ex[k];
                        mx[1] = mx[1] > ey[k] ? mx[1] : ey[k]; mn[1] = mn[1] < ey[k] ? mn[1] : ey[k];
                    }
                    have = true;
                }
            }
            if (have) flush(q);
            if (hit) rd[q] = 1;
        }
        int *pend_n = b.coll() + KD_COLL_PEND_N, *pend = b.coll() + KD_COLL_PEND;
        if (b.tid == 0) *pend_n = 0;
        b.sync();
        if (b.tid == 0) *live_n = 0;
        KDP(0);
        for (int q = b.tid; q < nr; q += b.nth) {
            if (rd[q] == 0) { rd[q] = -1; continue; }
            double shi[3], slo[3];
            for (int k = 0; k < 3; k++) {
                const float up = f32_unsortable(bbf[6 * q + k]), dn = f32_unsortable(bbf[6 * q + 3 + k]);
                shi[k] = (double)up - (double)dn;
                slo[k] = shi[k] - 2.0 * (f32_ulp(up) + f32_ulp(dn));
            }
            slo[2] = 0.0;
            int d = 0;
            if (shi[1] > shi[d]) d = 1;
            if (shi[2] > shi[d]) d = 2;
            bool sure = true;
            for (int k = 0; k < 3; k++) if (k != d && !(slo[d] > shi[k])) sure = false;
            if (!OCTA_UNLIKELY(!sure)) { rd[q] = (signed char)d; continue; }
            if ((int)re[q] - (int)rs[q] > 256) {
                const int slot = atomic_add_int(pend_n, 1);
                if (slot < 64) { pend[slot] = q; rd[q] = (signed char)-2; continue; }
            }
            double hi3[3] = {0, 0, 0}, lo3[3] = {0, 0, 0};
            for (int i = rs[q]; i < re[q]; i++) {
                const double *p = pts + 3 * (int)(kv[i] & KD_IDX_MASK);
                for (int k = 0; k < 3; k++) {
                    if (i == rs[q]) { hi3[k] = lo3[k] = p[k]; }
                    else { hi3[k] = hi3[k] > p[k] ? hi3[k] : p[k]; lo3[k] = lo3[k] < p[k] ? lo3[k] : p[k]; }
                }
            }
            d = 0;
            double size = 0;
            for (int k = 0; k < 3; k++) if (hi3[k] - lo3[k] > size) { d = k; size = hi3[k] - lo3[k]; }
            rd[q] = (hi3[d] == lo3[d]) ? (signed char)-1 : (signed char)d;
        }
// ... 638 lines not shown
        while (__ballot(fin != 0)) {
            const bool on = fin != 0;
            const int t = on ? (int)__ffs((int)fin) - 1 : 0;
            if (on) fin &= fin - 1u;
            double a = 0.5, k = 2.0;
#pragma unroll
            for (int e = 0; e < MURRAY_EPT; e++) if (t == e) { a = acc[e]; k = kk[e]; }
            if (!on) { a = 0.5; k = 2.0; }
            const double rp = octa_gpow::gpow_t(a, 1.0 / k, log_tab, exp_tab);
#pragma unroll
            for (int e = 0; e < MURRAY_EPT; e++)
                if (on && t == e) { *(volatile double *)(fl_val + (e * nw + w) * 64 + lane) = rp; rad[node[e]] = rp; pend[e] = 8; }
        }
        __builtin_amdgcn_wave_barrier();
        bool any = false;
        for (int e = 0; e < MURRAY_EPT; e++) {
            const unsigned long long fb = __ballot(pend[e] == 8);
            if (pend[e] == 8) pend[e] = 0;
            if (fb) {
                if (lane == 0) {
                    int *dw = fl_done + 2 * (e * nw + w);
                    __hip_atomic_fetch_or(dw, (int)(unsigned)fb, __ATOMIC_RELAXED, __HIP_MEMORY_SCOPE_WORKGROUP);
                    __hip_atomic_fetch_or(dw + 1, (int)(unsigned)(fb >> 32), __ATOMIC_RELAXED, __HIP_MEMORY_SCOPE_WORKGROUP);
                }
                done += (int)__popcll(fb);
                any = true;
            }
        }
        __builtin_amdgcn_wave_barrier();
        if (!any) __builtin_amdgcn_s_sleep(2);
    }
    return rounds;
}
#endif

OCTA_HD inline int murray_flush(const Blk &b, const SimArrays &A, int f, const SeqLds &L, int n_def) {
    if (n_def <= 0) return 0;
    int *ctl = b.coll() + 90;
    if (b.tid == 0) ctl[0] = 0;
    double *rad = L.rad;
    int rounds = 0;
#if defined(__HIP_DEVICE_COMPILE__)
    if (n_def <= MURRAY_EPT * 64) {
        static_assert(MURRAY_EPT * 64 <= MURRAY_FLUSH_LDS, "flush slots");
        if (b.tid < 64) {
            FlushRec *recs = A.fl_rec + (size_t)f * MURRAY_FLUSH_LDS;
            murray_flush_prepare_wave(A, f, L, n_def, recs);
            __builtin_amdgcn_wave_barrier();
            __threadfence_block();
            rounds = murray_flush_rounds_wave(rad, L.log_tab, L.exp_tab, L.fl_val, L.fl_done, recs, n_def);
        }
        b.sync();
        return rounds;
    }
#endif
    if (n_def <= MURRAY_EPT * b.nth) {
        int node[MURRAY_EPT], c0[MURRAY_EPT], c1[MURRAY_EPT];
        double kk[MURRAY_EPT], acc[MURRAY_EPT];
        int pend[MURRAY_EPT];
        for (int e = 0; e < MURRAY_EPT; e++) {
            const int idx = b.tid + e * b.nth;
            pend[e] = 0; node[e] = 0; c0[e] = c1[e] = 0; kk[e] = 1; acc[e] = 0;
            if (idx < n_def) {
                node[e] = A.act_list[idx];
                const WalkRec r = walk_load(A, f, node[e], false);
                c0[e] = r.c0; c1[e] = r.c1; kk[e] = r.k;
                pend[e] = 4 | (r.nch >= 1 ? 1 : 0) | (r.nch >= 2 ? 2 : 0);
            }
        }
        b.sync();
        while (true) {
            rounds++;
            int fin = 0;
            for (int e = 0; e < MURRAY_EPT; e++) {
                if (!(pend[e] & 4)) continue;
                if ((pend[e] & 1) && !deferred_get(L, c0[e])) { acc[e] = acc[e] + octa_gpow::gpow_t(rad[c0[e]], kk[e], L.log_tab, L.exp_tab); pend[e] &= ~1; }
                if ((pend[e] & 2) && !deferred_get(L, c1[e])) { acc[e] = acc[e] + octa_gpow::gpow_t(rad[c1[e]], kk[e], L.log_tab, L.exp_tab); pend[e] &= ~2; }
                if (!(pend[e] & 3)) {
                    rad[node[e]] = octa_gpow::gpow_t(acc[e], 1.0 / kk[e], L.log_tab, L.exp_tab);
                    pend[e] = 8;
                    fin++;
                }
            }
            b.sync();
            for (int e = 0; e < MURRAY_EPT; e++)
                if (pend[e] == 8) { atomic_and_int(&L.deferred[node[e] >> 5], (int)~(1u << (node[e] & 31))); pend[e] = 0; }
            if (fin) atomic_add_int(&ctl[0], fin);
            b.sync();
            if (ctl[0] >= n_def) break;
        }
    } else {
        b.sync();
        while (true) {
            rounds++;
            int fin = 0;
            for (int idx = b.tid; idx < n_def; idx += b.nth) {
                const int id = A.act_list[idx];
                if (id < 0 || !deferred_get(L, id)) continue;
                const WalkRec r = walk_load(A, f, id, false);
                if ((r.nch >= 1 && deferred_get(L, r.c0)) || (r.nch >= 2 && deferred_get(L, r.c1))) continue;
                double s = 0;
                if (r.nch >= 1) s = octa_gpow::gpow_t(rad[r.c0], r.k, L.log_tab, L.exp_tab);
                if (r.nch >= 2) s = s + octa_gpow::gpow_t(rad[r.c1], r.k, L.log_tab, L.exp_tab);
                rad[id] = octa_gpow::gpow_t(s, 1.0 / r.k, L.log_tab, L.exp_tab);
                A.act_list[idx] = -1 - id;
                fin++;
            }
            b.sync();
            for (int idx = b.tid; idx < n_def; idx += b.nth) {
                const int v = A.act_list[idx];
                if (v < 0 && v != (int)0x80000000) {
                    const int id = -1 - v;
                    atomic_and_int(&L.deferred[id >> 5], (int)~(1u << (id & 31)));
                    A.act_list[idx] = (int)0x80000000;
                }
            }
            if (fin) atomic_add_int(&ctl[0], fin);
            b.sync();
            if (ctl[0] >= n_def) break;
        }
    }
    b.sync();
    return rounds;
}

OCTA_HD inline int seq_add_node(const SimArrays &A, int f, int &n_nodes, V3 p, double r, int parent, int parent_nch,
                                double kappa, const SeqLds &L) {
    int id = n_nodes;
    if (OCTA_UNLIKELY(id >= NCAP)) { atomic_or_int(&A.sc->err, ERR_NODE_CAP); return -1; }
    n_nodes = id + 1;
    st3(A.npos_of(f) + 3 * id, p);
    A.nrad_of(f)[id] = r; A.nkap_of(f)[id] = kappa; A.npar_of(f)[id] = parent;
    L.par[id] = (idx_t)parent;
    A.nch0_of(f)[id] = -1; A.nch1_of(f)[id] = -1; A.nnch_of(f)[id] = 0; A.nact_of(f)[id] = 1;
    if (parent_nch == 0) A.nch0_of(f)[parent] = id; else if (parent_nch == 1) A.nch1_of(f)[parent] = id;
    A.nnch_of(f)[parent] = (unsigned char)(parent_nch + 1);
    return id;
}

OCTA_HD inline int add_node(const SimArrays &A, int f, V3 p, double r, int parent, double kappa, double *rad_mirror = nullptr) {
    int id = A.sc->n_nodes[f];
    if (OCTA_UNLIKELY(id >= NCAP)) { atomic_or_int(&A.sc->err, ERR_NODE_CAP); return -1; }
    A.sc->n_nodes[f] = id + 1;
    st3(A.npos_of(f) + 3 * id, p);
    A.nrad_of(f)[id] = r; A.nkap_of(f)[id] = kappa; A.npar_of(f)[id] = parent;
    if (rad_mirror) rad_mirror[id] = r;
    A.nch0_of(f)[id] = -1; A.nch1_of(f)[id] = -1; A.nnch_of(f)[id] = 0; A.nact_of(f)[id] = 1;
    if (parent >= 0) {
        int c = A.nnch_of(f)[parent];
        if (c == 0) A.nch0_of(f)[parent] = id; else if (c == 1) A.nch1_of(f)[parent] = id;
        A.nnch_of(f)[parent] = (unsigned char)(c + 1);
    }
    return id;
}

#if OCTA_SIM_LARGE || defined(OCTA_SIM_SAMPLE_DIRECT)
OCTA_HD inline void phase_sample(const Blk &b, const SimArrays &A, const SimConst &C, const IterParams &P, int iter) {
    SampleScalars *sc = A.sc;
    const int N = P.N;
    const double *cand = A.cand;
    (void)iter;
    const double en = fmax(P.eps_n, P.eps_k), es = P.eps_s;
    const double en2 = en * en;
    const float en_hi2f = nextafterf((float)((en + GRID_F_TAU) * (en + GRID_F_TAU)), INFINITY);
    const float es_lo2f = es > GRID_F_TAU ? nextafterf((float)((es - GRID_F_TAU) * (es - GRID_F_TAU)), -INFINITY) : 0.f;
    const float es_hi2f = nextafterf((float)((es + GRID_F_TAU) * (es + GRID_F_TAU)), INFINITY);
    const double GSd = C.gs;
    const double fcx = C.fc0 * GSd, fcy = C.fc1 * GSd, fr = sc->faz_radius * GSd * 0.5;
    int *vlist = A.tmp_int;
    int *plist = A.tmp_int + NCANDCAP;
#if defined(OCTA_SIM_PROF_SAMPLE) && defined(__HIP_DEVICE_COMPILE__)
    long _st = (long)wall_clock64();
#define SSP(slot) do { if (b.tid == 0) { long _t = (long)wall_clock64(); sc->kdprof[slot] += _t - _st; _st = _t; } } while (0)
#else
#define SSP(slot) do { } while (0)
#endif
    for (int i = b.tid; i < N; i += b.nth) {
        V3 p = ld3(cand + 3 * i);
        int ok = !(p.x >= C.sx || p.y >= C.sy || p.z >= C.sz || p.x < 0 || p.y < 0 || p.z < 0);
        if (ok && C.fixed) {
            const int vi = (int)(unsigned short)(int)(p.x * GSd), vj = (int)(unsigned short)(int)(p.y * GSd), vk = (int)(unsigned short)(int)(p.z * GSd);
            ok = vi < C.gshape[0] && vj < C.gshape[1] && vk < C.gshape[2] && C.mask[((size_t)vi * C.gshape[1] + vj) * C.gshape[2] + vk] != 0;
        } else if (ok) {
            double dd = sqrt((p.x - fcx) * (p.x - fcx) + (p.y - fcy) * (p.y - fcy));
            ok = dd > fr;
        }
        A.removed[i] = (unsigned char)ok;
    }
    b.sync();
    const int n_valid = ordered_compact(b, N, [&](int i) { return A.removed[i] != 0; }, [&](int i, int pos) { vlist[pos] = i; });
    b.sync();
    SSP(0);
    const int n_art = sc->n_nodes[0];
    const int n_oxy = sc->n_oxy;
    unsigned char *okf = A.removed;
    double *oxd = A.tmp_dbl;
    for (int i = b.tid; i < n_art; i += b.nth) oxd[i] = oxygen_distance(A.nrad[0][i], C.ps);
    {
        Grid G = grid_build(b, A, A.npos[0], nullptr, n_art, en, 1, true);
        SSP(1);
        for (int rep = 0; rep < ((OCTA_SIM_DUP & 8) ? 2 : 1); rep++)
        for (int vi = b.tid; vi < n_valid; vi += b.nth) {
            const V3 c = ld3(cand + 3 * vlist[vi]);
            bool ok = true;
            const float cxf = (float)c.x, cyf = (float)c.y, czf = (float)c.z;
            grid_visit_f(G, c.x, c.y, en, [&](int j, const Pt3f &qf) {
                if (ok) {
                    const float d2f = sqdist_f(qf, cxf, cyf, czf);
                    if (d2f <= en_hi2f) {
                        const double lim = fmin(en, oxd[j]), lo = lim - GRID_F_TAU, hi = lim + GRID_F_TAU;
                        if (lo > 0.0 && (double)d2f < lo * lo) ok = false;
                        else if (OCTA_UNLIKELY((double)d2f <= hi * hi)) {
                            const double d2 = sqdist(ld3(G.src + 3 * j), c);
                            if (d2 <= en2 && !(sqrt(d2) > oxd[j])) ok = false;
                        }
                    }
                }
            });
            okf[vi] = ok ? 1 : 0;
        }
        b.sync();
        SSP(2);
    }
    {
        Grid G = grid_build(b, A, A.oxy, nullptr, n_oxy, es, 1, true);
        SSP(3);
        for (int rep = 0; rep < ((OCTA_SIM_DUP & 8) ? 2 : 1); rep++)
        for (int vi = b.tid; vi < n_valid; vi += b.nth) {
            if (!okf[vi]) continue;
            V3 c = ld3(cand + 3 * vlist[vi]);
            bool ok = true;
            const float cxf = (float)c.x, cyf = (float)c.y, czf = (float)c.z;
            grid_visit_f(G, c.x, c.y, es, [&](int j, const Pt3f &qf) {
                if (ok) {
                    const float d2f = sqdist_f(qf, cxf, cyf, czf);
                    if (d2f < es_lo2f) ok = false;
                    else if (OCTA_UNLIKELY(d2f <= es_hi2f) && sqrt(sqdist(ld3(G.src + 3 * j), c)) <= es) ok = false;
                }
            });
            okf[vi] = ok ? 1 : 0;
        }
        b.sync();
        SSP(4);
    }
    const int n_pass = ordered_compact(b, n_valid, [&](int vi) { return okf[vi] != 0; }, [&](int vi, int pos) { plist[pos] = vlist[vi]; });
    b.sync();
    SSP(5);
#if defined(OCTA_SIM_PROF_SAMPLE) && defined(__HIP_DEVICE_COMPILE__)
    if (b.tid == 0) sc->kdprof[7] += n_pass;
#endif
    double *acc = reinterpret_cast<double *>(b.user_of<4>());
    int *ctl = b.coll() + 100;
    if (b.tid == 0) { ctl[0] = 0; ctl[1] = 0; ctl[2] = 0; }
    b.sync();
#if defined(__HIP_DEVICE_COMPILE__)
    constexpr int GP_MAX = 1024, GPAIR_CAP = 2048;
    static_assert((size_t)GP_MAX * 24 + (size_t)GP_MAX * 4 + (size_t)GPAIR_CAP * 2 + GP_MAX / 8 <= (size_t)SIM_USER_BYTES, "greedy acceptance tables");
    bool settled = false;
    if (n_pass <= GP_MAX) {
        double *pp = acc;
        unsigned short *rcnt = reinterpret_cast<unsigned short *>(pp + 3 * GP_MAX);
        unsigned short *rstart = rcnt + GP_MAX;
        unsigned short *pl = rstart + GP_MAX;
        unsigned *okb = reinterpret_cast<unsigned *>(pl + GPAIR_CAP);
        for (int q = b.tid; q < n_pass; q += b.nth) { st3(pp + 3 * q, ld3(cand + 3 * plist[q])); rcnt[q] = 0; }
        for (int w = b.tid; w < (n_pass + 31) / 32; w += b.nth) okb[w] = ~0u;
        b.sync();
        const double es2 = es * es, es2_lo = es2 * (1.0 - 1e-14), es2_hi = es2 * (1.0 + 1e-14);
        auto conflicts = [&](const V3 &c, int i) {
            const V3 d = sub(c, ld3(pp + 3 * i));
            const double s2 = (d.x * d.x + d.y * d.y) + d.z * d.z;
            if (s2 > es2_hi) return false;
            if (s2 < es2_lo) return true;
            return !(sqrt(s2) > es);
        };
        for (int t = b.tid; 2 * t < n_pass; t += b.nth) {
            for (int side = 0; side < 2; side++) {
                const int j = side == 0 ? t : n_pass - 1 - t;
                if (side == 1 && j == t) break;
                const V3 c = ld3(pp + 3 * j);
                int cnt = 0;
                {
                    int i = 0;
                    for (; i + 8 <= j; i += 8) {
                        V3 a[8];
#pragma unroll
                        for (int u = 0; u < 8; u++) a[u] = ld3(pp + 3 * (i + u));
#pragma unroll
                        for (int u = 0; u < 8; u++) {
                            const V3 d = sub(c, a[u]);
                            const double s2 = (d.x * d.x + d.y * d.y) + d.z * d.z;
                            if (!(s2 > es2_hi)) cnt += (s2 < es2_lo || !(sqrt(s2) > es)) ? 1 : 0;
                        }
                    }
                    for (; i < j; i++) cnt += conflicts(c, i) ? 1 : 0;
                }
                if (cnt > 0) {
                    const int at = atomic_add_int(&ctl[1], cnt);
                    if (at + cnt <= GPAIR_CAP) {
                        int w = at;
                        for (int i = 0; i < j; i++) if (conflicts(c, i)) pl[w++] = (unsigned short)i;
                        rstart[j] = (unsigned short)at; rcnt[j] = (unsigned short)cnt;
                    } else {
                        ctl[2] = 1;
                    }
                }
            }
        }
        b.sync();
        if (OCTA_UNI(ctl[2]) == 0) {
            settled = true;
            if (b.tid < 64) {
                const int lane = b.tid;
                for (int j0 = 0; j0 < n_pass; j0 += 64) {
                    unsigned long long m = __ballot(j0 + lane < n_pass && rcnt[j0 + lane] != 0);
                    while (m) {
                        const int j = j0 + (int)__ffsll((long long)m) - 1;
                        m &= m - 1ull;
                        const int s0 = rstart[j], c0 = rcnt[j];
                        bool hit = false;
                        for (int k = lane; k < c0; k += 64) { const int i = pl[s0 + k]; hit |= ((okb[i >> 5] >> (i & 31)) & 1u) != 0; }
                        if (__any(hit) && lane == 0) okb[j >> 5] &= ~(1u << (j & 31));
                        __builtin_amdgcn_wave_barrier();
                    }
                }
            }
            b.sync();
            const int room = OCAP - n_oxy < ACCCAP ? OCAP - n_oxy : ACCCAP;
            const int acc_all = ordered_compact(b, n_pass, [&](int q) { return ((okb[q >> 5] >> (q & 31)) & 1u) != 0; },
                                                [&](int q, int pos) { if (pos < room) st3(A.oxy + 3 * (size_t)(n_oxy + pos), ld3(pp + 3 * q)); });
            if (b.tid == 0) {
                if (acc_all > ACCCAP) atomic_or_int(&sc->err, ERR_ACC_CAP);
                ctl[0] = acc_all < ACCCAP ? acc_all : ACCCAP;
            }
        }
    }
    b.sync();
    if (!settled && b.tid < 64) {
        const int lane = b.tid;
        int acc_n = 0;
        for (int q0 = 0; q0 < n_pass; q0 += 64) {
            V3 mine = v3(0, 0, 0);
            if (q0 + lane < n_pass) mine = ld3(cand + 3 * plist[q0 + lane]);
            const int cnt = n_pass - q0 < 64 ? n_pass - q0 : 64;
            for (int jj = 0; jj < cnt; jj++) {
                const int jl = __builtin_amdgcn_readfirstlane(jj);
                const V3 c = v3(readlane_f64(mine.x, jl), readlane_f64(mine.y, jl), readlane_f64(mine.z, jl));
                bool conflict = false;
                for (int j = lane; j < acc_n; j += 64)
                    if (!(rownorm(sub(c, ld3(acc + 3 * j))) > es)) conflict = true;
                if (!__any(conflict)) {
                    if (acc_n < ACCCAP) { if (lane == 0) st3(acc + 3 * acc_n, c); }
                    else if (lane == 0) atomic_or_int(&sc->err, ERR_ACC_CAP);
                    acc_n++;
                    __builtin_amdgcn_wave_barrier();
                }
            }
        }
        if (lane == 0) ctl[0] = acc_n < ACCCAP ? acc_n : ACCCAP;
    }
#else
    {
        int acc_n = 0;
        for (int q = 0; q < n_pass; q++) {
            V3 c = ld3(cand + 3 * plist[q]);
            bool conflict = false;
            for (int j = 0; j < acc_n; j++)
                if (!(rownorm(sub(c, ld3(acc + 3 * j))) > es)) { conflict = true; break; }
            if (!conflict) {
                if (acc_n < ACCCAP) st3(acc + 3 * acc_n, c); else atomic_or_int(&sc->err, ERR_ACC_CAP);
                acc_n++;
            }
        }
        ctl[0] = acc_n < ACCCAP ? acc_n : ACCCAP;
    }
#endif
    b.sync();
    int acc_n = ctl[0];
    if (n_oxy + acc_n > OCAP) { if (b.tid == 0) atomic_or_int(&sc->err, ERR_OXY_CAP); acc_n = OCAP - n_oxy; }
#if defined(__HIP_DEVICE_COMPILE__)
    if (!settled)
#endif
    for (int j = b.tid; j < acc_n * 3; j += b.nth) A.oxy[3 * n_oxy + j] = acc[j];
    b.sync();
    if (b.tid == 0) sc->n_oxy = n_oxy + acc_n;
    b.sync();
    SSP(6);
#undef SSP
}
#else
#ifndef OCTA_SIM_SAMPLE_GRID
#define OCTA_SIM_SAMPLE_GRID 96
#endif
#ifndef OCTA_SIM_SAMPLE_NODE_FIRST
#define OCTA_SIM_SAMPLE_NODE_FIRST 0
#endif
constexpr int SMP_CH = 2048;
constexpr int SMP_GRID = OCTA_SIM_SAMPLE_GRID;
constexpr int SMP_GP_MAX = 1024, SMP_GPAIR_CAP = 2048;
constexpr size_t SMP_OFF_LIVE = (size_t)SMP_CH * 24, SMP_OFF_PP = SMP_OFF_LIVE + SMP_CH, SMP_OFF_SLOT = SMP_OFF_PP + (size_t)SMP_GP_MAX * 24;
static_assert(SMP_CH < 0xffff && SMP_GRID * SMP_GRID < 0xffff, "slots and cells are 16-bit, 0xffff marks a candidate that is not valid");
static_assert(SMP_OFF_PP + ((size_t)SMP_GRID * SMP_GRID + 2) / 2 * 4 <= SMP_OFF_SLOT && SMP_OFF_SLOT + (size_t)SMP_CH * 2 <= (size_t)SIM_USER_BYTES, "candidate grid layout");
static_assert((size_t)SMP_GP_MAX * 7 + (size_t)SMP_GPAIR_CAP * 2 <= SMP_OFF_LIVE && (size_t)ACCCAP * 24 <= SMP_OFF_PP + (size_t)SMP_GP_MAX * 24, "greedy acceptance tables");
#if defined(OCTA_SIM_SAMPLE_COUNT) && !defined(__HIP_DEVICE_COMPILE__)
static long smp_count[12];
static int smp_count_pass = 5;
#define SMP_COUNT(i, v) (smp_count[i] += (v))
#else
#define SMP_COUNT(i, v) ((void)0)
#endif
struct SmpGrid {
    int nc;
    double x0, inv;
    unsigned *endw;
    const double *pos;
    unsigned char *live;
};
OCTA_HD inline int smp_cell1(const SmpGrid &G, double x) { return grid_clampi((int)floor((x - G.x0) * G.inv), G.nc - 1); }
OCTA_HD inline int smp_end(const SmpGrid &G, int c) { return (int)((G.endw[c >> 1] >> ((c & 1) * 16)) & 0xffffu); }
template <class F>
OCTA_HD inline void smp_visit(const SmpGrid &G, double px, double py, double radius, F &&body) {
    const int cx0 = smp_cell1(G, px - radius), cx1 = smp_cell1(G, px + radius);
    const int cy0 = smp_cell1(G, py - radius), cy1 = smp_cell1(G, py + radius);
    for (int cyb = cy0; cyb <= cy1; cyb += 3) {
        int k0[3], k1[3];
#pragma unroll
        for (int r = 0; r < 3; r++) {
            const int row = cyb + r;
            k0[r] = k1[r] = 0;
            if (row <= cy1) {
                const int c0 = row * G.nc + cx0;
                k0[r] = c0 ? smp_end(G, c0 - 1) : 0;
                k1[r] = smp_end(G, row * G.nc + cx1);
            }
        }
#pragma unroll
        for (int r = 0; r < 3; r++) {
            for (int k = k0[r]; k < k1[r]; k += 2) {
                const int k2 = k + 1 < k1[r] ? k + 1 : k;
                const unsigned char l0 = G.live[k], l1 = G.live[k2];
                const V3 c0 = ld3(G.pos + 3 * k), c1 = ld3(G.pos + 3 * k2);
                SMP_COUNT(smp_count_pass, 1 + (k2 != k)); SMP_COUNT(smp_count_pass + 1, (l0 != 0) + (l1 && k2 != k));
                if (l0) body(k, c0);
                if (l1 && k2 != k) body(k2, c1);
            }
        }
    }
}
OCTA_HD inline void smp_settle(const Blk &b, int n, const unsigned short *rcnt, const unsigned short *rstart, const unsigned short *pl,
                               unsigned char *state, unsigned short *crow) {
#if defined(__HIP_DEVICE_COMPILE__)
    if (b.tid >= 64) return;
    const int lane = b.tid;
    int n_rows = 0;
    for (int j0 = 0; j0 < n; j0 += 64) {
        const bool c = j0 + lane < n && rcnt[j0 + lane] != 0;
        const unsigned long long m = __ballot(c);
        if (j0 + lane < n) state[j0 + lane] = c ? 0 : 1;
        if (c) crow[n_rows + (int)__popcll(m & ((1ull << lane) - 1ull))] = (unsigned short)(j0 + lane);
        n_rows += (int)__popcll(m);
    }
    __builtin_amdgcn_wave_barrier();
    asm volatile("" ::: "memory");
    const int step = 64;
#else
    const int lane = 0, step = 1;
    int n_rows = 0;
    for (int j = 0; j < n; j++) { state[j] = rcnt[j] ? 0 : 1; if (rcnt[j]) crow[n_rows++] = (unsigned short)j; }
#endif
    while (true) {
        bool left = false;
        for (int q = lane; q < n_rows; q += step) {
            const int j = crow[q];
            if (state[j]) continue;
            const int s0 = rstart[j], c0 = rcnt[j];
            bool hit = false, wait = false;
            for (int k = 0; k < c0; k++) { const int st = state[pl[s0 + k]]; hit |= st == 1; wait |= st == 0; }
            if (hit) state[j] = 2; else if (!wait) state[j] = 1; else left = true;
        }
#if defined(__HIP_DEVICE_COMPILE__)
        __builtin_amdgcn_wave_barrier();
        asm volatile("" ::: "memory");
        if (!__any(left)) break;
#else
        if (!left) break;
#endif
    }
}
OCTA_HD inline void phase_sample(const Blk &b, const SimArrays &A, const SimConst &C, const IterParams &P, int iter) {
    SampleScalars *sc = A.sc;
    const int N = P.N;
    const double *cand = A.cand;
    (void)iter;
    const double en = fmax(P.eps_n, P.eps_k), es = P.eps_s;
    const double en2 = en * en;
    const double es2 = es * es, es2_lo = es2 * (1.0 - 1e-14), es2_hi = es2 * (1.0 + 1e-14);
    const double GSd = C.gs;
    const double fcx = C.fc0 * GSd, fcy = C.fc1 * GSd, fr = sc->faz_radius * GSd * 0.5;
#if defined(OCTA_SIM_PROF_SAMPLE) && defined(__HIP_DEVICE_COMPILE__)
    long _st = (long)wall_clock64();
#define SSP(slot) do { b.sync(); if (b.tid == 0) { long _t = (long)wall_clock64(); sc->kdprof[slot] += _t - _st; _st = _t; } } while (0)
#else
#define SSP(slot) do { } while (0)
#endif
    unsigned char *const U = b.user_of<2>();
    double *const pos = reinterpret_cast<double *>(U);
    unsigned char *const live = U + SMP_OFF_LIVE;
    unsigned *const endw = reinterpret_cast<unsigned *>(U + SMP_OFF_PP);
    double *const pp = reinterpret_cast<double *>(U + SMP_OFF_PP);
    unsigned short *const slot_of = reinterpret_cast<unsigned short *>(U + SMP_OFF_SLOT);
    double *const ppg = A.tmp_dbl;
    const int n_art = sc->n_nodes[0];
    const int n_oxy = sc->n_oxy;
    const bool single = N <= SMP_CH;
    SmpGrid G;
    {
        const double cell = fmax(fmax(en, es), 1.2 / SMP_GRID);
        int nc = (int)ceil(1.2 / cell);
        G.nc = nc < 1 ? 1 : (nc > SMP_GRID ? SMP_GRID : nc);
        G.x0 = -0.1; G.inv = 1.0 / cell; G.endw = endw; G.pos = pos; G.live = live;
    }
    const int nc = G.nc, nwords = (nc * nc + 2) / 2;
    const double pad = 1e-9;
    int n_pass = 0;
    int *ctl = b.coll() + 100;
    SMP_COUNT(0, 1); SMP_COUNT(1, N); SMP_COUNT(3, n_art); SMP_COUNT(4, n_oxy);
    if (N <= 0) { b.sync(); if (b.tid == 0) { ctl[0] = 0; ctl[1] = 0; ctl[2] = 0; } }
    for (int base = 0; base < N; base += SMP_CH) {
        const int n = N - base < SMP_CH ? N - base : SMP_CH;
        b.sync();
        for (int w = b.tid; w < nwords; w += b.nth) endw[w] = 0;
        if (b.tid == 0) { ctl[0] = 0; ctl[1] = 0; ctl[2] = 0; }
        b.sync();
        for (int i = b.tid; i < n; i += b.nth) {
            const V3 p = ld3(cand + 3 * (size_t)(base + i));
            int ok = !(p.x >= C.sx || p.y >= C.sy || p.z >= C.sz || p.x < 0 || p.y < 0 || p.z < 0);
            if (ok && C.fixed) {
                const int vi = (int)(unsigned short)(int)(p.x * GSd), vj = (int)(unsigned short)(int)(p.y * GSd), vk = (int)(unsigned short)(int)(p.z * GSd);
                ok = vi < C.gshape[0] && vj < C.gshape[1] && vk < C.gshape[2] && C.mask[((size_t)vi * C.gshape[1] + vj) * C.gshape[2] + vk] != 0;
            } else if (ok) {
                double dd = sqrt((p.x - fcx) * (p.x - fcx) + (p.y - fcy) * (p.y - fcy));
                ok = dd > fr;
            }
            int c = 0xffff;
            if (ok) {
                SMP_COUNT(2, 1);
                c = smp_cell1(G, p.y) * nc + smp_cell1(G, p.x);
                atomic_add_int(reinterpret_cast<int *>(&endw[c >> 1]), 1 << ((c & 1) * 16));
            }
            slot_of[i] = (unsigned short)c;
        }
        b.sync();
        {
            const int chunk = ((nwords + b.nth - 1) / b.nth) | 1;
            const int w0 = b.tid * chunk < nwords ? b.tid * chunk : nwords, w1 = w0 + chunk < nwords ? w0 + chunk : nwords;
            int local = 0;
            for (int w = w0; w < w1; w++) { const unsigned v = endw[w]; local += (int)(v & 0xffffu) + (int)(v >> 16); }
            int ex;
            blk_scan(b, local, &ex);
            unsigned run = (unsigned)ex;
            for (int w = w0; w < w1; w++) {
                const unsigned v = endw[w], lo = v & 0xffffu, hi = v >> 16;
                endw[w] = run | ((run + lo) << 16);
                run += lo + hi;
            }
        }
        b.sync();
        for (int i = b.tid; i < n; i += b.nth) {
            const int c = slot_of[i];
            if (c != 0xffff) {
                const V3 p = ld3(cand + 3 * (size_t)(base + i));
                const int sh = (c & 1) * 16;
                const int k = (int)(((unsigned)atomic_add_int(reinterpret_cast<int *>(&endw[c >> 1]), 1 << sh) >> sh) & 0xffffu);
                st3(pos + 3 * k, p);
                live[k] = 1;
                slot_of[i] = (unsigned short)k;
            }
        }
        b.sync();
        SSP(0);
        constexpr int SB = 4;
        auto sink_pass = [&]() {
            for (int i0 = b.tid; i0 < n_oxy; i0 += SB * b.nth) {
                V3 s[SB];
#pragma unroll
                for (int u = 0; u < SB; u++) { const int i = i0 + u * b.nth; s[u] = ld3(A.oxy + 3 * (size_t)(i < n_oxy ? i : n_oxy - 1)); }
                OCTA_ISSUE_LOADS();
#pragma unroll
                for (int u = 0; u < SB; u++)
                    if (i0 + u * b.nth < n_oxy)
                        smp_visit(G, s[u].x, s[u].y, es + pad, [&](int k, const V3 &c) {
                            const double d2 = sqdist(s[u], c);
                            if (!(d2 > es2_hi) && (d2 < es2_lo || sqrt(d2) <= es)) live[k] = 0;
                        });
            }
            SSP(4);
        };
        auto node_pass = [&]() {
            for (int i0 = b.tid; i0 < n_art; i0 += SB * b.nth) {
                V3 q[SB];
                double rad[SB];
#pragma unroll
                for (int u = 0; u < SB; u++) {
                    const int i = i0 + u * b.nth, ic = i < n_art ? i : n_art - 1;
                    q[u] = ld3(A.npos[0] + 3 * (size_t)ic);
                    rad[u] = A.nrad[0][ic];
                }
                OCTA_ISSUE_LOADS();
#pragma unroll
                for (int u = 0; u < SB; u++)
                    if (i0 + u * b.nth < n_art) {
                        const double oxd = oxygen_distance(rad[u], C.ps);
                        const double lim = oxd < en ? oxd : en;
                        const double o2 = oxd * oxd, o2_lo = o2 * (1.0 - 1e-14), o2_hi = o2 * (1.0 + 1e-14);
                        smp_visit(G, q[u].x, q[u].y, lim + pad, [&](int k, const V3 &c) {
                            const double d2 = sqdist(q[u], c);
                            if (d2 <= en2 && !(d2 > o2_hi) && (d2 < o2_lo || !(sqrt(d2) > oxd))) live[k] = 0;
                        });
                    }
            }
            SSP(2);
        };
        for (int rep = 0; rep < ((OCTA_SIM_DUP & 8) ? 2 : 1); rep++) {
#if defined(OCTA_SIM_SAMPLE_COUNT) && !defined(__HIP_DEVICE_COMPILE__)
            auto count_live = [&]() { for (int i = 0; i < n; i++) if (slot_of[i] != 0xffff && live[slot_of[i]]) SMP_COUNT(9, 1); };
            smp_count_pass = OCTA_SIM_SAMPLE_NODE_FIRST ? 7 : 5;
#if OCTA_SIM_SAMPLE_NODE_FIRST
            node_pass(); count_live(); smp_count_pass = 5; sink_pass();
#else
            sink_pass(); count_live(); smp_count_pass = 7; node_pass();
#endif
#elif OCTA_SIM_SAMPLE_NODE_FIRST
            node_pass(); sink_pass();
#else
            sink_pass(); node_pass();
#endif
        }
        b.sync();
        auto passes = [&](int i) { const int k = slot_of[i]; return k != 0xffff && live[k] != 0; };
        const int n_cp = ordered_compact(b, n, passes, [&](int i, int at) {
            const V3 p = ld3(pos + 3 * (int)slot_of[i]);
            if (single) { if (at < SMP_GP_MAX) st3(pp + 3 * at, p); }
            else st3(ppg + 3 * (size_t)(n_pass + at), p);
        });
        if (single && n_cp > SMP_GP_MAX) {
            b.sync();
            ordered_compact(b, n, passes, [&](int i, int at) { st3(ppg + 3 * (size_t)at, ld3(pos + 3 * (int)slot_of[i])); });
        }
        n_pass += n_cp;
    }
    b.sync();
    bool in_hbm = !single || n_pass > SMP_GP_MAX;
    SSP(5);
#if defined(OCTA_SIM_PROF_SAMPLE) && defined(__HIP_DEVICE_COMPILE__)
    if (b.tid == 0) sc->kdprof[7] += n_pass;
#endif
    double *acc = reinterpret_cast<double *>(b.user_of<4>());
    bool settled = false;
    int acc_n = 0;
    if (n_pass <= SMP_GP_MAX) {
        unsigned short *rcnt = reinterpret_cast<unsigned short *>(U);
        unsigned short *rstart = rcnt + SMP_GP_MAX;
        unsigned short *crow = rstart + SMP_GP_MAX;
        unsigned short *pl = crow + SMP_GP_MAX;
        unsigned char *state = reinterpret_cast<unsigned char *>(pl + SMP_GPAIR_CAP);
        if (!single) {
            for (int j = b.tid; j < 3 * n_pass; j += b.nth) pp[j] = ppg[j];
            b.sync();
        }
        auto conflicts = [&](const V3 &c, int i) {
            const V3 d = sub(c, ld3(pp + 3 * i));
            const double s2 = (d.x * d.x + d.y * d.y) + d.z * d.z;
            if (s2 > es2_hi) return false;
            if (s2 < es2_lo) return true;
// ... 963 lines not shown
#if defined(__HIP_DEVICE_COMPILE__)
    else {
        static_assert(SIM_THREADS_PER_WG == 256, "the ordered pass hands its side work to waves 1 - 3");
        const int wv = b.tid >> 6;
        if (wv == 1) side(side_lds);
        const int nw = (f == 1 || pend_other > 2 * MURRAY_FLUSH_WAVE) ? 3 : 2;
        const int w = wv == 2 ? 0 : (wv == 3 ? 1 : 2);
        if (w < nw && w * 64 < pend_other) {
            const int rounds = murray_flush_rounds_wave(A.nrad_of(1 - f), L.log_tab, L.exp_tab, L.fl_val, L.fl_done, A.fl_rec + (size_t)(1 - f) * MURRAY_FLUSH_LDS,
                                                        pend_other, w, nw, true);
            if (b.tid == 128) sc->flush_rounds += rounds;
        }
    }
#else
    (void)side; (void)side_lds;
#endif
#undef SEQT
#undef SEQ2_TOP
#undef SEQ2_SEL
#undef SEQ2_END
#undef SEQ2_ARG
    b.sync();
#if defined(__HIP_DEVICE_COMPILE__)
    if (b.tid == 0 && pend_other > 0) sc->fl_pending[1 - f] = 0;
#endif
    {
        long t0 = OCTA_FLUSH_T0();
        const int rounds = murray_flush(b, A, f, L, b.coll()[91]);
        if (b.tid == 0) {
            sc->kdprof[7] += OCTA_FLUSH_T0() - t0; sc->flush_rounds += rounds;
#if defined(OCTA_SIM_PROF_SEQ) && defined(__HIP_DEVICE_COMPILE__)
            sc->kdprof[3] += OCTA_FLUSH_T0() - t0;
#endif
        }
    }
    b.sync();
}

OCTA_HD inline void murray_flush_pending(const Blk &b, const SimArrays &A) {
#if defined(__HIP_DEVICE_COMPILE__)
    b.sync();
    double *fl_val = reinterpret_cast<double *>(b.user_of<8>());
    int *fl_done = reinterpret_cast<int *>(fl_val + MURRAY_FLUSH_LDS);
    for (int f = 0; f < 2; f++) {
        const int n = OCTA_UNI(A.sc->fl_pending[f]);
        if (n <= 0) continue;
        for (int i = b.tid; i < MURRAY_FLUSH_LDS / 32; i += b.nth) fl_done[i] = 0;
        b.sync();
        const int wv = b.tid >> 6;
        if (wv < 3 && wv * 64 < n) {
            const int rounds = murray_flush_rounds_wave(A.nrad_of(f), octa_gpow::LOG_TAB, octa_gpow::EXP_TAB, fl_val, fl_done, A.fl_rec + (size_t)f * MURRAY_FLUSH_LDS, n,
                                                        wv, 3, true);
            if (b.tid == 0) { A.sc->fl_pending[f] = 0; A.sc->flush_rounds += rounds; }
        }
        b.sync();
    }
#else
    (void)b; (void)A;
#endif
}

constexpr int COMPACT_TILE = 3072;
constexpr int COMPACT_TILE_NN = 2048;
OCTA_HD inline int compact_points(const Blk &b, double *pts, int n, const unsigned char *removed, double *stage, int *c_nn = nullptr,
                                  double *c_d2 = nullptr) {
    (void)stage;
    if (b.nth == 1) {
        int w = 0;
        for (int i = 0; i < n; i++)
            if (!removed[i]) {
                if (w != i) {
                    pts[3 * w] = pts[3 * i]; pts[3 * w + 1] = pts[3 * i + 1]; pts[3 * w + 2] = pts[3 * i + 2];
                    if (c_nn) { c_nn[w] = c_nn[i]; c_d2[w] = c_d2[i]; }
                }
                w++;
            }
        return w;
    }
    double *tile = reinterpret_cast<double *>(b.user_of<16>());
    static_assert((size_t)COMPACT_TILE * 24 <= (size_t)SIM_USER_BYTES && (size_t)COMPACT_TILE_NN * 36 <= (size_t)SIM_USER_BYTES, "compaction tile");
#if defined(__HIP_DEVICE_COMPILE__)
    const int lane = b.tid & 63, wv = b.tid >> 6, nw = (b.nth + 63) >> 6;
    const int TILE = c_nn ? COMPACT_TILE_NN : COMPACT_TILE;
    double *td = tile + 3 * COMPACT_TILE_NN;
    int *ti = reinterpret_cast<int *>(td + COMPACT_TILE_NN);
    int base = 0;
    for (int t0 = 0; t0 < n; t0 += TILE) {
        const int tn = n - t0 < TILE ? n - t0 : TILE;
        const int seg = ((tn + nw * 64 - 1) / (nw * 64)) * 64;
        const int s0 = t0 + (wv * seg < tn ? wv * seg : tn), s1 = s0 + seg < t0 + tn ? s0 + seg : t0 + tn;
        int c = 0;
        for (int i0 = s0; i0 < s1; i0 += 64) c += (int)__popcll(__ballot(i0 + lane < s1 && !removed[i0 + lane]));
        int ex;
        const int kept = blk_scan(b, lane == 0 ? c : 0, &ex);
        if (base != t0 || kept != tn) {
            int at = __builtin_amdgcn_readfirstlane(ex);
            constexpr int CB = 2;
            for (int i0 = s0; i0 < s1; i0 += CB * 64) {
                bool keep[CB];
                V3 v[CB];
                int vn[CB] = {};
                double vd[CB] = {};
#pragma unroll
                for (int u = 0; u < CB; u++) {
                    const int i = i0 + u * 64 + lane, ic = i < s1 ? i : s1 - 1;
                    keep[u] = i < s1 && !removed[ic];
                    v[u] = ld3(pts + 3 * (size_t)ic);
                    if (c_nn) { vn[u] = c_nn[ic]; vd[u] = c_d2[ic]; }
                }
                OCTA_ISSUE_LOADS();
#pragma unroll
                for (int u = 0; u < CB; u++) {
                    const unsigned long long m = __ballot(keep[u]);
                    if (keep[u]) {
                        const int w = at + (int)__popcll(m & ((1ull << lane) - 1ull));
                        tile[3 * w] = v[u].x; tile[3 * w + 1] = v[u].y; tile[3 * w + 2] = v[u].z;
                        if (c_nn) { ti[w] = vn[u]; td[w] = vd[u]; }
                    }
                    at += (int)__popcll(m);
                }
            }
            b.sync();
            for (int j = b.tid; j < kept * 3; j += b.nth) pts[(size_t)3 * base + j] = tile[j];
            if (c_nn)
                for (int j = b.tid; j < kept; j += b.nth) { c_nn[base + j] = ti[j]; c_d2[base + j] = td[j]; }
            b.sync();
        }
        base += kept;
    }
    return base;
#else
    (void)tile;
    return n;
#endif
}

OCTA_HD inline bool assign_memory_covers(const SimArrays &A, int f, int n) {
#ifdef OCTA_SIM_ASSIGN_NOCACHE
    (void)A; (void)f; (void)n;
    return false;
#else
    return OCTA_UNI((int)(A.nn_prev_of(f) != nullptr && A.sc->n_cached[f] == n)) != 0;
#endif
}

#if defined(__HIP_DEVICE_COMPILE__)
#define OCTA_SUBPROF(sc, slot, t0) do { if (b.tid == 0) { long _t1 = (long)wall_clock64(); (sc)->prof[slot] += _t1 - (t0); (t0) = _t1; } } while (0)
#define OCTA_SUBPROF_T0() ((long)wall_clock64())
#else
#define OCTA_SUBPROF(sc, slot, t0) do { (void)(t0); } while (0)
#define OCTA_SUBPROF_T0() 0L
#endif

OCTA_HD inline void phase_satisfy_art(const Blk &b, const SimArrays &A, const SimConst &C, const IterParams &P) {
    const double zext = C.sz;
    SampleScalars *sc = A.sc;
    const int nb = sc->new_begin[0], ne = sc->new_end[0];
    const int n_new = ne - nb, n_oxy = sc->n_oxy;
    if (n_new <= 0 || n_oxy <= 0) return;
    const double ek = P.eps_k, ek2 = ek * ek;
    long t0 = OCTA_SUBPROF_T0();
    for (int i = b.tid; i < n_oxy; i += b.nth) A.removed[i] = 0;
    int *ctl = b.coll() + 100;
    if (b.tid == 0) { ctl[0] = 0; ctl[1] = 0; ctl[2] = 0; }
    unsigned char *xf = reinterpret_cast<unsigned char *>(A.nn);
    static_assert((size_t)NCAP <= (size_t)OCAP * sizeof(int), "group flags fit the nearest-node list");
    for (int j = b.tid; j < n_new && j < NCAP; j += b.nth) xf[j] = 0;
    b.sync();
    {
        int *new_ids = A.tmp_int;
        for (int j = b.tid; j < n_new; j += b.nth) new_ids[j] = nb + j;
        b.sync();
        Grid G = grid_build(b, A, A.npos[0], new_ids, n_new, ek);
        for (int o = b.tid; o < n_oxy; o += b.nth) {
            const V3 p = ld3(A.oxy + 3 * o);
            grid_visit(G, p.x, p.y, ek, [&](int j, const V3 &q) {
                if (sqdist(p, q) <= ek2) {
                    int slot = atomic_add_int(&ctl[0], 1);
                    if (slot < PCAP) A.pairs[slot] = ((unsigned)(j - nb) << IDX_BITS) | (unsigned)o;
                    A.removed[o] = 1;
                }
            });
        }
        b.sync();
    }
    OCTA_SUBPROF(sc, 12, t0);
    int n_pairs = ctl[0];
    if (n_pairs > PCAP) { if (b.tid == 0) atomic_or_int(&sc->err, ERR_PAIR_CAP); n_pairs = PCAP; }
    if (n_new > (1 << (32 - IDX_BITS))) { if (b.tid == 0) atomic_or_int(&sc->err, ERR_PAIR_CAP); }
    b.sync();
    if (n_pairs == 0) return;
    {
        const int n_ven = sc->n_nodes[1];
        int *rem = A.tmp_int;
        int n_rem = 0;
        {
            const int chunk = (n_oxy + b.nth - 1) / b.nth;
            const int i0 = b.tid * chunk < n_oxy ? b.tid * chunk : n_oxy, i1 = (i0 + chunk < n_oxy) ? i0 + chunk : n_oxy;
            int local = 0;
            for (int o = i0; o < i1; o++) local += A.removed[o] ? 1 : 0;
            int ex;
            n_rem = blk_scan(b, local, &ex);
            int run = ex;
            for (int o = i0; o < i1; o++) if (A.removed[o]) rem[run++] = o;
        }
        b.sync();
        for (int k = b.tid; k < n_rem; k += b.nth) {
            const int o = rem[k];
            A.ven_near[o] = 0;
            A.hashes[o] = py_hash_tuple3(ld3(A.oxy + 3 * o));
        }
        Grid G = grid_build(b, A, A.oxy, rem, n_rem, ek);
        constexpr int VB = 4;
        for (int j0 = b.tid; j0 < n_ven; j0 += VB * b.nth) {
            V3 qv[VB];
#pragma unroll
            for (int u = 0; u < VB; u++) { const int j = j0 + u * b.nth; qv[u] = ld3(A.npos[1] + 3 * (j < n_ven ? j : n_ven - 1)); }
#pragma unroll
            for (int u = 0; u < VB; u++) {
                if (j0 + u * b.nth >= n_ven) break;
                const V3 q = qv[u];
                grid_visit(G, q.x, q.y, ek, [&](int o, const V3 &p) {
                    if (sqrt(sqdist(q, p)) <= ek) A.ven_near[o] = 1;
                });
            }
        }
        b.sync();
    }
    OCTA_SUBPROF(sc, 12, t0);
    bool set_in_lds = false;
    int rung = 0;
    bool from_partial = false;
    auto sink_of = [&](unsigned pr) -> int {
        const unsigned low = pr & IDX_MASK;
        return (rung == 2 || (rung == 1 && xf[pr >> IDX_BITS])) ? (int)A.kd_idx[low] : (int)low;
    };
#ifdef OCTA_SIM_DEBUG_SAT
    int dbg_n_ins = -1, dbg_mask = -1, dbg_base = -1;
    const int dbg_n_co2_in = sc->n_co2;
#endif
    while (true) {
        const int vslot = rung == 1 ? 2 : 1;
        if (rung > 0) {
            if (rung == 1) {
                for (int i = b.tid; i < n_pairs; i += b.nth) {
                    const unsigned pr = A.pairs[i];
                    if (xf[pr >> IDX_BITS]) A.removed[pr & IDX_MASK] = 3;
                }
            } else if (OCTA_UNLIKELY(from_partial)) {
                for (int i = b.tid; i < n_pairs; i += b.nth) {
                    const unsigned pr = A.pairs[i];
                    if (xf[pr >> IDX_BITS]) A.pairs[i] = (pr & ~IDX_MASK) | (unsigned)A.kd_idx[pr & IDX_MASK];
                }
            }
            b.sync();
            const unsigned char need_bits = rung == 1 ? (unsigned char)2 : (unsigned char)0xff;
            kd_build(b, A.oxy, n_oxy, A.kd_idx, A.kd_rank, reinterpret_cast<float *>(A.tmp_dbl), 0.0, zext, sc->kdprof, A.removed, true, need_bits);
#if OCTA_SIM_DUP & 1
            kd_build(b, A.oxy, n_oxy, A.kd_idx, A.kd_rank, reinterpret_cast<float *>(A.tmp_dbl), 0.0, zext, nullptr, A.removed, true, need_bits);
#endif
            for (int i = b.tid; i < n_pairs; i += b.nth) {
                unsigned pr = A.pairs[i];
                if (rung == 2 || xf[pr >> IDX_BITS]) A.pairs[i] = (pr & ~IDX_MASK) | (unsigned)A.kd_rank[pr & IDX_MASK];
            }
            b.sync();
            OCTA_SUBPROF(sc, 11, t0);
        }
        unsigned *keys = reinterpret_cast<unsigned *>(b.user_of<32>());
        int n_pow2 = 1;
        while (n_pow2 < n_pairs) n_pow2 <<= 1;
        for (int i = b.tid; i < n_pow2; i += b.nth) keys[i] = i < n_pairs ? A.pairs[i] : 0xffffffffu;
        b.sync();
        if (n_pairs > 0) blk_sort_u32(b, keys, n_pow2);
        for (int i = b.tid; i < n_pairs; i += b.nth) A.pairs[i] = keys[i];
        b.sync();
        OCTA_SUBPROF(sc, 13, t0);
#if defined(__HIP_DEVICE_COMPILE__)
#if defined(OCTA_SIM_PROF_SET)
        long _pt = (long)wall_clock64();
#define PSP(slot) do { if (b.tid == 0) { long _t = (long)wall_clock64(); sc->kdprof[slot] += _t - _pt; _pt = _t; } } while (0)
#else
#define PSP(slot) do { } while (0)
#endif
        constexpr int EMPTY = 0x7fffffff;
        auto replay = [&](int *own, int *in_key, unsigned long long *in_hash, int *dk, unsigned long long *dh, int *ord0, int *ord1,
                          const int s_max) __attribute__((always_inline)) -> int {
            int n_ins = 0;
            for (int p0 = 0; p0 < n_pairs; p0 += b.nth) {
                const int i = p0 + b.tid;
                int o = -1, take = 0;
                unsigned long long hsh = 0;
                if (i < n_pairs) {
                    o = sink_of(keys[i]);
                    take = A.ven_near[o] ? 0 : 1;
                    hsh = A.hashes[o];
                }
                int ex;
                const int tot = blk_scan(b, take, &ex);
                if (take) { in_key[n_ins + ex] = (int)((keys[i] & ~IDX_MASK) | (unsigned)o); in_hash[n_ins + ex] = hsh; }
                n_ins += tot;
            }
            b.sync();
            PSP(0);
            for (int i = b.tid; i < n_ins; i += b.nth) own[(unsigned)in_key[i] & IDX_MASK] = EMPTY;
            b.sync();
            for (int i = b.tid; i < n_ins; i += b.nth) atomic_min_int(&own[(unsigned)in_key[i] & IDX_MASK], i);
            b.sync();
            int D = 0;
            for (int p0 = 0; p0 < n_ins; p0 += b.nth) {
                const int i = p0 + b.tid;
                const bool first = i < n_ins && own[(unsigned)in_key[i] & IDX_MASK] == i;
                int ex;
                const int tot = blk_scan(b, first ? 1 : 0, &ex);
                if (first) { dk[D + ex] = in_key[i]; dh[D + ex] = in_hash[i]; }
                D += tot;
            }
            b.sync();
            PSP(1);
            int S = 8, n_prev = 0;
            int *ord = ord0, *ord_next = ord1;
            while (true) {
                const int thr = (3 * (S - 1) + 4) / 5;
                const int upto = D < thr ? D : thr;
                const unsigned long long mask = (unsigned long long)(S - 1);
                for (int p = n_prev + b.tid; p < upto; p += b.nth) ord[p] = p;
                for (int e = b.tid; e < S; e += b.nth) own[e] = EMPTY;
                b.sync();
                for (int p = b.tid; p < upto; p += b.nth) {
                    int cur = p;
                    unsigned long long hsh = dh[ord[cur]], i = hsh & mask, perturb = hsh;
                    int lin = 0, nlin = (i + 9 <= mask) ? 9 : 0;
                    auto next = [&] {
                        if (lin < nlin) { lin++; return; }
                        perturb >>= 5;
                        i = (i * 5 + 1 + perturb) & mask;
                        nlin = (i + 9 <= mask) ? 9 : 0; lin = 0;
                    };
                    while (true) {
                        const int slot = (int)i + lin;
                        const int old = atomic_min_ret_int(&own[slot], cur);
                        if (old == EMPTY) break;
                        if (old > cur) {
                            cur = old;
                            hsh = dh[ord[cur]]; i = hsh & mask; perturb = hsh; lin = 0; nlin = (i + 9 <= mask) ? 9 : 0;
                            while ((int)i + lin != slot) next();
                        }
                        next();
                    }
                }
                b.sync();
                if (rung < 2) {
                    for (int p = n_prev + b.tid; p < upto; p += b.nth) {
                        const unsigned g = (unsigned)dk[p] >> IDX_BITS;
                        if (rung == 1 && xf[g]) continue;
                        const unsigned long long hsh = dh[p];
                        unsigned long long i = hsh & mask, perturb = hsh;
                        int lin = 0, nlin = (i + 9 <= mask) ? 9 : 0;
                        while (true) {
                            const int q = own[(int)i + lin];
                            if (q == p) break;
                            if (q == EMPTY || (q >= n_prev && ((unsigned)dk[q] >> IDX_BITS) == g)) {
                                if (rung == 0) xf[g] = 1;
                                atomic_or_int(&ctl[vslot], 1);
                                break;
                            }
                            if (lin < nlin) { lin++; continue; }
                            perturb >>= 5;
                            i = (i * 5 + 1 + perturb) & mask;
                            nlin = (i + 9 <= mask) ? 9 : 0; lin = 0;
                        }
                    }
                    if (b.tid == 0 && D > thr && ((unsigned)dk[thr - 1] >> IDX_BITS) == ((unsigned)dk[thr] >> IDX_BITS)) {
                        const unsigned g = (unsigned)dk[thr] >> IDX_BITS;
                        if (rung == 0) { xf[g] = 1; atomic_or_int(&ctl[vslot], 1); }
                        else if (!xf[g]) atomic_or_int(&ctl[vslot], 1);
                    }
#ifdef OCTA_SIM_KD_PARTIAL_REFUSE
                    if (b.tid == 0 && rung == 1) atomic_or_int(&ctl[vslot], 1);
#endif
                    b.sync();
                    if (rung == 1 && OCTA_UNLIKELY(ctl[vslot])) break;
                }
// ... 46 lines not shown
            unsigned long long *dh = in_hash + LSET_PAIRS;
            static_assert((size_t)(OWN_N + 4 * LSET_PAIRS + 1) * 4 + (size_t)2 * LSET_PAIRS * 8 <= (size_t)SIM_USER_BYTES, "set replay layout");
            static_assert((size_t)LSET_PAIRS * 4 <= (size_t)OWN_N * 4, "the sorted pairs (start of the table area) end before the insert stream");
            mask = replay(own, in_key, in_hash, dk, dh, ord0, ord1, S_MAX);
            t_key = own;
            set_in_lds = true;
        } else if (HBM_REPLAY && n_pairs <= PCAP) {
            int *own = A.set_key;
            int *in_key = A.tmp_int, *ord0 = A.tmp_int + PCAP;
            unsigned long long *in_hash = A.set_hash;
            unsigned long long *dh = reinterpret_cast<unsigned long long *>(A.tmp_dbl);
            int *dk = reinterpret_cast<int *>(A.tmp_dbl + OCAP), *ord1 = dk + OCAP;
            mask = replay(own, in_key, in_hash, dk, dh, ord0, ord1, SETCAP / 2);
            t_key = own;
            set_in_lds = true;
        }
        if (set_in_lds && (rung == 2 || !ctl[vslot])) {
            const int n_co2_0 = sc->n_co2;
            int base = 0;
            {
                const int per = (mask + 1 + b.nth - 1) / b.nth;
                const int e0 = b.tid * per < mask + 1 ? b.tid * per : mask + 1, e1 = e0 + per < mask + 1 ? e0 + per : mask + 1;
                int cnt = 0;
                for (int e = e0; e < e1; e++) cnt += t_key[e] >= 0 ? 1 : 0;
                int ex2;
                base = blk_scan(b, cnt, &ex2);
                int dst = n_co2_0 + ex2;
                constexpr int RB = 8;
                for (int eb = e0; eb < e1; eb += RB) {
                    int k[RB];
                    V3 v[RB];
#pragma unroll
                    for (int u = 0; u < RB; u++) { k[u] = eb + u < e1 ? t_key[eb + u] : -1; }
#pragma unroll
                    for (int u = 0; u < RB; u++) v[u] = ld3(A.oxy + 3 * (k[u] >= 0 ? k[u] : 0));
#pragma unroll
                    for (int u = 0; u < RB; u++)
                        if (k[u] >= 0) { if (dst < CCAP) st3(A.co2 + 3 * dst, v[u]); dst++; }
                }
            }
            b.sync();
            PSP(4);
            if (b.tid == 0) {
                int n_co2 = n_co2_0 + base;
                if (n_co2 > CCAP) { sc->err |= ERR_CO2_CAP; n_co2 = CCAP; }
                sc->n_co2 = n_co2;
            }
#ifdef OCTA_SIM_DEBUG_SAT
            dbg_mask = mask; dbg_base = base;
#endif
        }
#undef PSP
#endif
        if (!set_in_lds && b.tid == 0) {
            PySetView S;
            S.hash = A.set_hash; S.key = A.set_key; S.err = &sc->err; S.cap = SETCAP;
            pyset_init(S);
            int *cw = reinterpret_cast<int *>(A.tmp_dbl);
            static_assert((size_t)SETCAP / 2 <= (size_t)2 * OCAP, "certificate table");
            int D = 0;
            for (int i = 0; i < n_pairs; i++) {
                const unsigned pr = A.pairs[i];
                const int o = sink_of(pr);
                if (!A.ven_near[o]) {
                    const int used = S.used;
                    pyset_add(S, o, A.hashes[o]);
                    if (rung < 2 && S.used != used) { cw[D] = o; cw[OCAP + D] = (int)(pr >> IDX_BITS); D++; }
                }
            }
            if (rung < 2 && pyset_order_check(cw, cw + OCAP, A.hashes, D, cw + 4 * OCAP, cw + 2 * OCAP, cw + 3 * OCAP, SETCAP / 2, xf, rung == 1)) ctl[vslot] = 1;
#ifdef OCTA_SIM_KD_PARTIAL_REFUSE
            if (rung == 1) ctl[vslot] = 1;
#endif
            if (rung == 2 || !ctl[vslot]) {
                int n_co2 = sc->n_co2;
                for (int e = 0; e <= S.mask; e++)
                    if (S.key[e] >= 0) {
                        if (n_co2 >= CCAP) { sc->err |= ERR_CO2_CAP; break; }
                        int o = S.key[e];
                        A.co2[3 * n_co2] = A.oxy[3 * o]; A.co2[3 * n_co2 + 1] = A.oxy[3 * o + 1]; A.co2[3 * n_co2 + 2] = A.oxy[3 * o + 2];
                        n_co2++;
                    }
                sc->n_co2 = n_co2;
            }
        }
        b.sync();
        OCTA_SUBPROF(sc, 14, t0);
        if (rung < 2 && ctl[vslot]) {
#ifdef OCTA_SIM_KD_NOPARTIAL
            rung = 2;
#else
            from_partial = rung == 1;
            rung++;
#endif
            continue;
        }
        if (b.tid == 0) sc->kd_path[rung]++;
        break;
    }
#if defined(OCTA_SIM_DEBUG_SAT) && !defined(OCTA_SIM_ITER_PROF)
    {
        int ex, loc;
        loc = 0; for (int o = b.tid; o < n_oxy; o += b.nth) loc += A.removed[o] ? 1 : 0;
        const int c_rem = blk_scan(b, loc, &ex);
        loc = 0; for (int o = b.tid; o < n_oxy; o += b.nth) loc += (A.removed[o] && A.ven_near[o]) ? 1 : 0;
        const int c_ven = blk_scan(b, loc, &ex);
        unsigned char *mark = reinterpret_cast<unsigned char *>(A.tmp_dbl);
        for (int o = b.tid; o < 2 * n_oxy; o += b.nth) mark[o] = 0;
        b.sync();
        for (int i = b.tid; i < n_pairs; i += b.nth) {
            const int o = sink_of(A.pairs[i]);
            mark[o] = 1;
            if (!A.ven_near[o]) mark[n_oxy + o] = 1;
        }
        b.sync();
        loc = 0; for (int o = b.tid; o < n_oxy; o += b.nth) loc += mark[o];
        const int c_pair_all = blk_scan(b, loc, &ex);
        loc = 0; for (int o = b.tid; o < n_oxy; o += b.nth) loc += mark[n_oxy + o];
        const int c_pair_take = blk_scan(b, loc, &ex);
        loc = 0; for (int o = b.tid; o < n_oxy; o += b.nth) loc += (mark[o] != (A.removed[o] ? 1 : 0)) ? 1 : 0;
        const int c_pair_vs_removed = blk_scan(b, loc, &ex);
        int c_slots = -1, c_in_distinct = -1, c_slot_bad = -1;
        if (set_in_lds) {
            const int *t_key = reinterpret_cast<const int *>(b.user());
            const int *in_key = t_key + (OCAP > LSET_CAP / 2 ? OCAP : LSET_CAP / 2);
            loc = 0; for (int e = b.tid; e <= dbg_mask; e += b.nth) loc += t_key[e] >= 0 ? 1 : 0;
            c_slots = blk_scan(b, loc, &ex);
            loc = 0; for (int e = b.tid; e <= dbg_mask; e += b.nth) { const int k = t_key[e]; if (k >= 0 && (k >= n_oxy || !A.removed[k] || A.ven_near[k])) loc++; }
            c_slot_bad = blk_scan(b, loc, &ex);
            for (int o = b.tid; o < n_oxy; o += b.nth) mark[o] = 0;
            b.sync();
            for (int i = b.tid; i < dbg_n_ins; i += b.nth) { const int k = (int)((unsigned)in_key[i] & IDX_MASK); if (k < n_oxy) mark[k] = 1; }
            b.sync();
            loc = 0; for (int o = b.tid; o < n_oxy; o += b.nth) loc += mark[o];
            c_in_distinct = blk_scan(b, loc, &ex);
        }
        b.sync();
        if (b.tid == 0 && A.dbg) {
            int *row = A.dbg + 16 * A.dbg_it;
            row[0] = n_new; row[1] = n_oxy; row[2] = n_pairs; row[3] = c_rem; row[4] = c_ven; row[5] = c_pair_all; row[6] = c_pair_take;
            row[7] = c_pair_vs_removed; row[8] = dbg_n_ins; row[9] = dbg_mask; row[10] = dbg_base; row[11] = c_slots; row[12] = c_in_distinct;
            row[13] = c_slot_bad; row[14] = dbg_n_co2_in; row[15] = sc->n_co2;
        }
        b.sync();
    }
#endif
    const bool carry = assign_memory_covers(A, 0, n_oxy);
    int keep = compact_points(b, A.oxy, n_oxy, A.removed, A.tmp_dbl, carry ? A.nn_prev[0] : nullptr, carry ? A.nn_d2[0] : nullptr);
    if (b.tid == 0) { sc->n_oxy = keep; sc->n_cached[0] = carry ? keep : 0; }
    b.sync();
    OCTA_SUBPROF(sc, 15, t0);
}

OCTA_HD inline void phase_satisfy_ven(const Blk &b, const SimArrays &A, const IterParams &P) {
    SampleScalars *sc = A.sc;
    const int nb = sc->new_begin[1], ne = sc->new_end[1];
    const int n_new = ne - nb, n_co2 = sc->n_co2;
    if (n_new <= 0 || n_co2 <= 0) return;
    const double ek2 = P.eps_k * P.eps_k;
    const double ek = P.eps_k;
    {
        int *new_ids = A.tmp_int;
        for (int j = b.tid; j < n_new; j += b.nth) new_ids[j] = nb + j;
        b.sync();
        Grid G = grid_build(b, A, A.npos[1], new_ids, n_new, ek);
        for (int o = b.tid; o < n_co2; o += b.nth) {
            const V3 p = ld3(A.co2 + 3 * o);
            bool hit = false;
            grid_visit(G, p.x, p.y, ek, [&](int, const V3 &q) {
                if (!hit && sqdist(p, q) <= ek2) hit = true;
            });
            A.removed[o] = hit ? 1 : 0;
        }
        b.sync();
    }
    const bool carry = assign_memory_covers(A, 1, n_co2);
    int keep = compact_points(b, A.co2, n_co2, A.removed, A.tmp_dbl, carry ? A.nn_prev[1] : nullptr, carry ? A.nn_d2[1] : nullptr);
    if (b.tid == 0) { sc->n_co2 = keep; sc->n_cached[1] = carry ? keep : 0; }
    b.sync();
}

}
```

Measured before the change: 1528.

## Replace global-memory grid in satisfy phases with LDS-binned chunked spatial grid

The satisfy phases (arterial sink removal, venous flagging, CO2 source removal) now bin the smaller point set in chunks into an LDS-resident uniform grid with packed 16-bit cell end offsets, then stream the larger set against it. This replaces the global-memory grid_build/grid_visit path, which remains available behind a compile flag. The aim is to cut global-memory traffic and atomics during neighbour queries. It also records removed sink ids in LDS so the later venous pass can skip a compaction scan. A standalone test entry point and profiling counters are added. The risks are chunking overhead when the binned set is large and the 16-bit limits on slot and cell indices.

```diff
diff --git a/include/octa_hip.h b/include/octa_hip.h
--- a/include/octa_hip.h
+++ b/include/octa_hip.h
@@ -316,6 +316,10 @@
                         double *h_oxy, int64_t n_oxy, int64_t cap_oxy, double eps_n, double eps_k, double eps_s, const double *h_cst8,
                         int64_t *h_n_out);
 
+int octa_sim_kat_satisfy_hits(octa_ctx *ctx, const double *h_new, int64_t n_new, const double *h_oxy, int64_t n_oxy, const double *h_ven, int64_t n_ven,
+                              const double *h_co2, int64_t n_co2, double eps_k, uint32_t *h_pairs, int64_t cap_pairs, uint8_t *h_removed,
+                              uint8_t *h_ven_near, uint64_t *h_hashes, uint8_t *h_co2_flags, int64_t *h_info3);
+
 #ifdef __cplusplus
 }
 #endif
diff --git a/octa_autosegmentation_amd/_native.py b/octa_autosegmentation_amd/_native.py
--- a/octa_autosegmentation_amd/_native.py
+++ b/octa_autosegmentation_amd/_native.py
@@ -148,6 +148,7 @@
     "octa_sim_kat_kd_order_signflag": (c_int, [c_void_p, c_void_p, ctypes.c_int64, c_void_p, ctypes.c_int32, c_void_p]),
     "octa_sim_kat_sample": (c_int, [c_void_p, c_void_p, ctypes.c_int64, c_void_p, c_void_p, ctypes.c_int64, c_void_p, ctypes.c_int64, ctypes.c_int64,
                                     c_double, c_double, c_double, c_void_p, c_void_p]),
+    "octa_sim_kat_satisfy_hits": (c_int, [c_void_p] + [c_void_p, ctypes.c_int64] * 4 + [c_double, c_void_p, ctypes.c_int64] + [c_void_p] * 5),
 }
 
 
diff --git a/octa_autosegmentation_amd/csrc/sim.hip b/octa_autosegmentation_amd/csrc/sim.hip
--- a/octa_autosegmentation_amd/csrc/sim.hip
+++ b/octa_autosegmentation_amd/csrc/sim.hip
@@ -38,6 +38,7 @@
 #define octa_sim_kat_kd_order OCTA_SIM_FN(kat_kd_order)
 #define octa_sim_kat_kd_order_signflag OCTA_SIM_FN(kat_kd_order_signflag)
 #define octa_sim_kat_sample OCTA_SIM_FN(kat_sample)
+#define octa_sim_kat_satisfy_hits OCTA_SIM_FN(kat_satisfy_hits)
 struct OCTA_SIM_T;
 extern "C" void octa_sim_destroy(OCTA_SIM_T *S);
 extern "C" long long octa_sim_next_ticket(void);
@@ -1374,6 +1375,86 @@
     Blk b = {(int)threadIdx.x, (int)blockDim.x, smem};
     phase_sample(b, A, C, P, 0);
 }
+
+__global__ void __launch_bounds__(SIM_THREADS)
+sim_kat_satisfy_kernel(SimArrays A, SimArrays A2, IterParams P, int *out2) {
+    extern __shared__ __attribute__((aligned(16))) unsigned char smem[];
+    Blk b = {(int)threadIdx.x, (int)blockDim.x, smem};
+    const SampleScalars *sc = A.sc;
+    const int n_new = sc->new_end[0] - sc->new_begin[0];
+    int n_pairs = 0;
+    if (n_new > 0 && sc->n_oxy > 0) {
+        long t0 = 0;
+        n_pairs = satisfy_art_hits(b, A, P, t0);
+        if (b.tid == 0) { out2[0] = (b.coll() + 100)[0]; out2[1] = n_pairs; }
+    }
+    b.sync();
+    if (n_new > 0 && sc->n_co2 > 0) satisfy_ven_flags(b, A2, P);
+}
+}
+
+extern "C" int octa_sim_kat_satisfy_hits(octa_ctx *ctx, const double *h_new, int64_t n_new, const double *h_oxy, int64_t n_oxy, const double *h_ven, int64_t n_ven,
+                                         const double *h_co2, int64_t n_co2, double eps_k, uint32_t *h_pairs, int64_t cap_pairs, uint8_t *h_removed,
+                                         uint8_t *h_ven_near, uint64_t *h_hashes, uint8_t *h_co2_flags, int64_t *h_info3) {
+    constexpr int NB = 3;
+    if (!ctx || !h_info3 || n_new < 0 || n_new + NB > NCAP || n_oxy < 0 || n_oxy > OCAP || n_ven < 0 || n_ven > NCAP || n_co2 < 0 || n_co2 > CCAP || cap_pairs < 0 ||
+        (n_new && !h_new) || (n_oxy && (!h_oxy || !h_removed || !h_ven_near || !h_hashes)) || (n_ven && !h_ven) || (n_co2 && (!h_co2 || !h_co2_flags)) ||
+        (cap_pairs && !h_pairs)) {
+        octa::set_error("octa_sim_kat_satisfy_hits: bad arguments");
+        return -2;
+    }
+    OCTA_HIP_CHECK(hipSetDevice(ctx->device));
+    SampleScalars sc;
+    memset(&sc, 0, sizeof(sc));
+    sc.n_nodes[0] = NB + (int)n_new; sc.n_nodes[1] = (int)n_ven; sc.n_oxy = (int)n_oxy; sc.n_co2 = (int)n_co2;
+    sc.new_begin[0] = sc.new_begin[1] = NB; sc.new_end[0] = sc.new_end[1] = NB + (int)n_new;
+    IterParams P;
+    memset(&P, 0, sizeof(P));
+    P.eps_k = eps_k;
+    const size_t n_dbl = (size_t)NCAP * 3 * 2 + (size_t)OCAP * 3 + (size_t)CCAP * 3 + (size_t)GRID_N * 3;
+    const size_t off_hash = n_dbl * 8, off_pairs = off_hash + (size_t)OCAP * 8, off_int = off_pairs + (size_t)PCAP * 4;
+    const size_t off_nn = off_int + ((size_t)OCAP + 2 * (size_t)NCANDCAP) * 4, off_byte = off_nn + (size_t)OCAP * 4;
+    const size_t off_sc = (off_byte + 3 * (size_t)OCAP + 15) & ~(size_t)15, off_out = off_sc + ((sizeof(SampleScalars) + 15) & ~(size_t)15);
+    unsigned char *d = nullptr;
+    OCTA_HIP_CHECK(hipMalloc(&d, off_out + 16));
+    int rc = 0;
+    auto ok = [&](hipError_t e, const char *what) { if (e != hipSuccess && rc == 0) { octa::set_error("octa_sim_kat_satisfy_hits: %s: %s", what, hipGetErrorString(e)); rc = -1; } return rc == 0; };
+    double *dd = reinterpret_cast<double *>(d);
+    SimArrays A;
+    memset((void *)&A, 0, sizeof(A));
+    A.npos[0] = dd; A.npos[1] = dd + (size_t)NCAP * 3; A.oxy = A.npos[1] + (size_t)NCAP * 3; A.co2 = A.oxy + (size_t)OCAP * 3; A.grid_pts = A.co2 + (size_t)CCAP * 3;
+    A.hashes = reinterpret_cast<unsigned long long *>(d + off_hash); A.pairs = reinterpret_cast<unsigned *>(d + off_pairs);
+    A.tmp_int = reinterpret_cast<int *>(d + off_int); A.nn = reinterpret_cast<int *>(d + off_nn);
+    A.removed = d + off_byte; A.ven_near = A.removed + OCAP; A.sc = reinterpret_cast<SampleScalars *>(d + off_sc);
+    SimArrays A2 = A;
+    A2.npos[1] = A.npos[0]; A2.removed = A.ven_near + OCAP;
+    int *d_out = reinterpret_cast<int *>(d + off_out);
+    int out2[2] = {0, 0};
+    if (ok(hipMemset(d, 0, off_out + 16), "clear") && ok(hipMemset(A.ven_near, 7, OCAP), "fill") &&
+        (!n_new || ok(hipMemcpy(A.npos[0] + 3 * NB, h_new, sizeof(double) * 3 * n_new, hipMemcpyHostToDevice), "new nodes")) &&
+        (!n_ven || ok(hipMemcpy(A.npos[1], h_ven, sizeof(double) * 3 * n_ven, hipMemcpyHostToDevice), "venous nodes")) &&
+        (!n_oxy || ok(hipMemcpy(A.oxy, h_oxy, sizeof(double) * 3 * n_oxy, hipMemcpyHostToDevice), "sinks")) &&
+        (!n_co2 || ok(hipMemcpy(A.co2, h_co2, sizeof(double) * 3 * n_co2, hipMemcpyHostToDevice), "sources")) &&
+        ok(hipMemcpy(A.sc, &sc, sizeof(sc), hipMemcpyHostToDevice), "scalars") &&
+        ok(hipFuncSetAttribute(reinterpret_cast<const void *>(sim_kat_satisfy_kernel), hipFuncAttributeMaxDynamicSharedMemorySize, (int)SIM_LDS), "attribute")) {
+        hipLaunchKernelGGL(sim_kat_satisfy_kernel, dim3(1), dim3(SIM_THREADS), SIM_LDS, 0, A, A2, P, d_out);
+        if (ok(hipGetLastError(), "launch") && ok(hipMemcpy(&sc, A.sc, sizeof(sc), hipMemcpyDeviceToHost), "result") &&
+            ok(hipMemcpy(out2, d_out, sizeof(out2), hipMemcpyDeviceToHost), "counts")) {
+            const int n_pairs = out2[1] < 0 ? 0 : (out2[1] > PCAP ? PCAP : out2[1]);
+            std::vector<unsigned> pairs(n_pairs);
+            if ((!n_pairs || ok(hipMemcpy(pairs.data(), A.pairs, sizeof(unsigned) * n_pairs, hipMemcpyDeviceToHost), "pairs")) &&
+                (!n_oxy || (ok(hipMemcpy(h_removed, A.removed, n_oxy, hipMemcpyDeviceToHost), "removed") &&
+                            ok(hipMemcpy(h_ven_near, A.ven_near, n_oxy, hipMemcpyDeviceToHost), "venous flags") &&
+                            ok(hipMemcpy(h_hashes, A.hashes, sizeof(unsigned long long) * n_oxy, hipMemcpyDeviceToHost), "hashes"))) &&
+                (!n_co2 || ok(hipMemcpy(h_co2_flags, A2.removed, n_co2, hipMemcpyDeviceToHost), "source flags"))) {
+                std::sort(pairs.begin(), pairs.end());
+                for (int64_t k = 0; k < n_pairs && k < cap_pairs; k++) h_pairs[k] = pairs[k];
+                h_info3[0] = sc.err; h_info3[1] = out2[0]; h_info3[2] = n_pairs;
+            }
+        }
+    }
+    (void)hipFree(d);
+    return rc;
 }
 
 extern "C" int octa_sim_kat_sample(octa_ctx *ctx, const double *h_cand, int64_t n_cand, const double *h_npos, const double *h_nrad, int64_t n_art,
diff --git a/octa_autosegmentation_amd/csrc/sim_api.cpp b/octa_autosegmentation_amd/csrc/sim_api.cpp
--- a/octa_autosegmentation_amd/csrc/sim_api.cpp
+++ b/octa_autosegmentation_amd/csrc/sim_api.cpp
@@ -32,6 +32,8 @@
 int octa_simS_kat_kd_order_signflag(octa_ctx *, const double *, int64_t, const uint8_t *, int32_t, int32_t *);
 int octa_simS_kat_sample(octa_ctx *, const double *, int64_t, const double *, const double *, int64_t, double *, int64_t, int64_t, double, double, double,
                          const double *, int64_t *);
+int octa_simS_kat_satisfy_hits(octa_ctx *, const double *, int64_t, const double *, int64_t, const double *, int64_t, const double *, int64_t, double,
+                               uint32_t *, int64_t, uint8_t *, uint8_t *, uint64_t *, uint8_t *, int64_t *);
 }
 
 #include <atomic>
@@ -124,4 +126,9 @@
                                    int64_t n_oxy, int64_t cap_oxy, double eps_n, double eps_k, double eps_s, const double *cst8, int64_t *n_out) {
     return octa_simS_kat_sample(ctx, cand, n_cand, npos, nrad, n_art, oxy, n_oxy, cap_oxy, eps_n, eps_k, eps_s, cst8, n_out);
 }
+extern "C" int octa_sim_kat_satisfy_hits(octa_ctx *ctx, const double *newp, int64_t n_new, const double *oxy, int64_t n_oxy, const double *ven, int64_t n_ven,
+                                         const double *co2, int64_t n_co2, double eps_k, uint32_t *pairs, int64_t cap_pairs, uint8_t *removed,
+                                         uint8_t *ven_near, uint64_t *hashes, uint8_t *co2_flags, int64_t *info3) {
+    return octa_simS_kat_satisfy_hits(ctx, newp, n_new, oxy, n_oxy, ven, n_ven, co2, n_co2, eps_k, pairs, cap_pairs, removed, ven_near, hashes, co2_flags, info3);
+}
 extern "C" int octa_sim_is_large(const octa_sim *sim) { return sim && sim->large ? 1 : 0; }
diff --git a/octa_autosegmentation_amd/csrc/sim_core.h b/octa_autosegmentation_amd/csrc/sim_core.h
--- a/octa_autosegmentation_amd/csrc/sim_core.h
+++ b/octa_autosegmentation_amd/csrc/sim_core.h
@@ -957,7 +957,7 @@
 OCTA_HD inline void kd_build(const Blk &b, const double *pts, int n, idx_t *out_idx, idx_t *out_rank,
                               float *xy, double zlo, double zhi, long *kdprof = nullptr, const unsigned char *need = nullptr,
                               const bool flag_in_sign = false, const unsigned char need_bits = 0xff) {
-#if defined(__HIP_DEVICE_COMPILE__) && !defined(OCTA_SIM_PROF_ASSIGN) && !defined(OCTA_SIM_PROF_SAMPLE) && !defined(OCTA_SIM_PROF_SET) && !defined(OCTA_SIM_PROF_MAIL) && !defined(OCTA_SIM_PROF_SEQ) && !defined(OCTA_SIM_PROF_SEQ2)
+#if defined(__HIP_DEVICE_COMPILE__) && !defined(OCTA_SIM_PROF_ASSIGN) && !defined(OCTA_SIM_PROF_SAMPLE) && !defined(OCTA_SIM_PROF_SET) && !defined(OCTA_SIM_PROF_MAIL) && !defined(OCTA_SIM_PROF_SEQ) && !defined(OCTA_SIM_PROF_SEQ2) && !defined(OCTA_SIM_PROF_SATISFY)
 #define KDP(slot) do { if (kdprof && b.tid == 0) { long _t = (long)wall_clock64(); kdprof[slot] += _t - _kt; _kt = _t; } } while (0)
     long _kt = (long)wall_clock64();
 #else
@@ -1902,6 +1902,127 @@
         A.nnch_of(f)[parent] = (unsigned char)(c + 1);
     }
     return id;
+}
+
+#ifndef OCTA_SIM_SAMPLE_GRID
+#define OCTA_SIM_SAMPLE_GRID 96
+#endif
+constexpr int SMP_GRID = OCTA_SIM_SAMPLE_GRID;
+#if defined(OCTA_SIM_SAMPLE_COUNT) && !defined(__HIP_DEVICE_COMPILE__)
+static long smp_count[12];
+static int smp_count_pass = 5;
+#define SMP_COUNT(i, v) (smp_count[i] += (v))
+#else
+#define SMP_COUNT(i, v) ((void)0)
+#endif
+#if defined(OCTA_SIM_SATISFY_COUNT) && !defined(__HIP_DEVICE_COMPILE__)
+static long sat_count[16], sat_max[16];
+static int sat_count_pass = 13;
+#define SAT_COUNT(i, v) do { const long _v = (long)(v); sat_count[i] += _v; if (_v > sat_max[i]) sat_max[i] = _v; } while (0)
+#define SAT_VISITED(n) (sat_count[sat_count_pass] += (n))
+#else
+#define SAT_COUNT(i, v) ((void)0)
+#define SAT_VISITED(n) ((void)0)
+#endif
+struct SmpGrid {
+    int nc;
+    double x0, inv;
+    unsigned *endw;
+    const double *pos;
+    unsigned char *live;
+};
+OCTA_HD inline void smp_setup(SmpGrid &G, double radius, int max_cells = SMP_GRID) {
+    const double cell = fmax(radius, 1.2 / max_cells);
+    const int nc = (int)ceil(1.2 / cell);
+    G.nc = nc < 1 ? 1 : (nc > max_cells ? max_cells : nc);
+    G.x0 = -0.1; G.inv = 1.0 / cell;
+}
+OCTA_HD inline int smp_cell1(const SmpGrid &G, double x) { return grid_clampi((int)floor((x - G.x0) * G.inv), G.nc - 1); }
+OCTA_HD inline int smp_end(const SmpGrid &G, int c) { return (int)((G.endw[c >> 1] >> ((c & 1) * 16)) & 0xffffu); }
+template <bool LIVE = true, class F>
+OCTA_HD inline void smp_visit(const SmpGrid &G, double px, double py, double radius, F &&body) {
+    const int cx0 = smp_cell1(G, px - radius), cx1 = smp_cell1(G, px + radius);
+    const int cy0 = smp_cell1(G, py - radius), cy1 = smp_cell1(G, py + radius);
+    for (int cyb = cy0; cyb <= cy1; cyb += 3) {
+        int k0[3], k1[3];
+#pragma unroll
+        for (int r = 0; r < 3; r++) {
+            const int row = cyb + r;
+            k0[r] = k1[r] = 0;
+            if (row <= cy1) {
+                const int c0 = row * G.nc + cx0;
+                k0[r] = c0 ? smp_end(G, c0 - 1) : 0;
+                k1[r] = smp_end(G, row * G.nc + cx1);
+            }
+        }
+#pragma unroll
+        for (int r = 0; r < 3; r++) {
+            constexpr int kstep = LIVE ? 2 : 1;
+            for (int k = k0[r]; k < k1[r]; k += kstep) {
+                const int k2 = (kstep == 2 && k + 1 < k1[r]) ? k + 1 : k;
+                const unsigned char l0 = LIVE ? G.live[k] : 1, l1 = LIVE ? G.live[k2] : 1;
+                const V3 c0 = ld3(G.pos + 3 * k), c1 = ld3(G.pos + 3 * k2);
+                if (LIVE) { SMP_COUNT(smp_count_pass, 1 + (k2 != k)); SMP_COUNT(smp_count_pass + 1, (l0 != 0) + (l1 && k2 != k)); }
+                else SAT_VISITED(1 + (k2 != k));
+                if (l0) body(k, c0);
+                if (l1 && k2 != k) body(k2, c1);
+            }
+        }
+    }
+}
+OCTA_HD inline void sat_bin(const Blk &b, const SmpGrid &G, double *pos, unsigned short *slot_id, unsigned short *cell_of, const double *pts,
+                            const unsigned short *ids, int id_base, int n) {
+    const int nc = G.nc, nwords = (nc * nc + 2) / 2;
+    unsigned *const endw = G.endw;
+    for (int i = b.tid; i < n; i += b.nth) {
+        const int c = smp_cell1(G, pts[3 * (size_t)i + 1]) * nc + smp_cell1(G, pts[3 * (size_t)i]);
+        atomic_add_int(reinterpret_cast<int *>(&endw[c >> 1]), 1 << ((c & 1) * 16));
+        cell_of[i] = (unsigned short)c;
+    }
+    b.sync();
+    {
+        const int chunk = ((nwords + b.nth - 1) / b.nth) | 1;
+        const int w0 = b.tid * chunk < nwords ? b.tid * chunk : nwords, w1 = w0 + chunk < nwords ? w0 + chunk : nwords;
+        int local = 0;
+        for (int w = w0; w < w1; w++) { const unsigned v = endw[w]; local += (int)(v & 0xffffu) + (int)(v >> 16); }
+        int ex;
+        blk_scan(b, local, &ex);
+        unsigned run = (unsigned)ex;
+        for (int w = w0; w < w1; w++) {
+            const unsigned v = endw[w], lo = v & 0xffffu, hi = v >> 16;
+            endw[w] = run | ((run + lo) << 16);
+            run += lo + hi;
+        }
+    }
+    b.sync();
+    for (int i = b.tid; i < n; i += b.nth) {
+        const int c = cell_of[i], sh = (c & 1) * 16;
+        const V3 p = ld3(pts + 3 * (size_t)i);
+        const int k = (int)(((unsigned)atomic_add_int(reinterpret_cast<int *>(&endw[c >> 1]), 1 << sh) >> sh) & 0xffffu);
+        st3(pos + 3 * k, p);
+        slot_id[k] = ids ? ids[i] : (unsigned short)(id_base + i);
+    }
+    b.sync();
+}
+template <class T, class D>
+OCTA_HD inline void sat_stream(const Blk &b, const SmpGrid &G, const double *pts, int n, double radius, T &&test, D &&done) {
+    constexpr int SB = 4;
+    const double box = radius + 1e-9;
+    for (int i0 = b.tid; i0 < n; i0 += SB * b.nth) {
+        V3 p[SB];
+#pragma unroll
+        for (int u = 0; u < SB; u++) { const int i = i0 + u * b.nth; p[u] = ld3(pts + 3 * (size_t)(i < n ? i : n - 1)); }
+        OCTA_ISSUE_LOADS();
+#pragma unroll
+        for (int u = 0; u < SB; u++) {
+            const int i = i0 + u * b.nth;
+            if (i < n) {
+                bool hit = false;
+                smp_visit<false>(G, p[u].x, p[u].y, box, [&](int k, const V3 &q) { if (test(i, p[u], k, q)) hit = true; });
+                done(i, p[u], hit);
+            }
+        }
+    }
 }
 
 #if OCTA_SIM_LARGE || defined(OCTA_SIM_SAMPLE_DIRECT)
@@ -2139,64 +2260,15 @@
 #undef SSP
 }
 #else
-#ifndef OCTA_SIM_SAMPLE_GRID
-#define OCTA_SIM_SAMPLE_GRID 96
-#endif
 #ifndef OCTA_SIM_SAMPLE_NODE_FIRST
 #define OCTA_SIM_SAMPLE_NODE_FIRST 0
 #endif
 constexpr int SMP_CH = 2048;
-constexpr int SMP_GRID = OCTA_SIM_SAMPLE_GRID;
 constexpr int SMP_GP_MAX = 1024, SMP_GPAIR_CAP = 2048;
 constexpr size_t SMP_OFF_LIVE = (size_t)SMP_CH * 24, SMP_OFF_PP = SMP_OFF_LIVE + SMP_CH, SMP_OFF_SLOT = SMP_OFF_PP + (size_t)SMP_GP_MAX * 24;
 static_assert(SMP_CH < 0xffff && SMP_GRID * SMP_GRID < 0xffff, "slots and cells are 16-bit, 0xffff marks a candidate that is not valid");
 static_assert(SMP_OFF_PP + ((size_t)SMP_GRID * SMP_GRID + 2) / 2 * 4 <= SMP_OFF_SLOT && SMP_OFF_SLOT + (size_t)SMP_CH * 2 <= (size_t)SIM_USER_BYTES, "candidate grid layout");
 static_assert((size_t)SMP_GP_MAX * 7 + (size_t)SMP_GPAIR_CAP * 2 <= SMP_OFF_LIVE && (size_t)ACCCAP * 24 <= SMP_OFF_PP + (size_t)SMP_GP_MAX * 24, "greedy acceptance tables");
-#if defined(OCTA_SIM_SAMPLE_COUNT) && !defined(__HIP_DEVICE_COMPILE__)
-static long smp_count[12];
-static int smp_count_pass = 5;
-#define SMP_COUNT(i, v) (smp_count[i] += (v))
-#else
-#define SMP_COUNT(i, v) ((void)0)
-#endif
-struct SmpGrid {
-    int nc;
-    double x0, inv;
-    unsigned *endw;
-    const double *pos;
-    unsigned char *live;
-};
-OCTA_HD inline int smp_cell1(const SmpGrid &G, double x) { return grid_clampi((int)floor((x - G.x0) * G.inv), G.nc - 1); }
-OCTA_HD inline int smp_end(const SmpGrid &G, int c) { return (int)((G.endw[c >> 1] >> ((c & 1) * 16)) & 0xffffu); }
-template <class F>
-OCTA_HD inline void smp_visit(const SmpGrid &G, double px, double py, double radius, F &&body) {
-    const int cx0 = smp_cell1(G, px - radius), cx1 = smp_cell1(G, px + radius);
-    const int cy0 = smp_cell1(G, py - radius), cy1 = smp_cell1(G, py + radius);
-    for (int cyb = cy0; cyb <= cy1; cyb += 3) {
-        int k0[3], k1[3];
-#pragma unroll
-        for (int r = 0; r < 3; r++) {
-            const int row = cyb + r;
-            k0[r] = k1[r] = 0;
-            if (row <= cy1) {
-                const int c0 = row * G.nc + cx0;
-                k0[r] = c0 ? smp_end(G, c0 - 1) : 0;
-                k1[r] = smp_end(G, row * G.nc + cx1);
-            }
-        }
-#pragma unroll
-        for (int r = 0; r < 3; r++) {
-            for (int k = k0[r]; k < k1[r]; k += 2) {
-                const int k2 = k + 1 < k1[r] ? k + 1 : k;
-                const unsigned char l0 = G.live[k], l1 = G.live[k2];
-                const V3 c0 = ld3(G.pos + 3 * k), c1 = ld3(G.pos + 3 * k2);
-                SMP_COUNT(smp_count_pass, 1 + (k2 != k)); SMP_COUNT(smp_count_pass + 1, (l0 != 0) + (l1 && k2 != k));
-                if (l0) body(k, c0);
-                if (l1 && k2 != k) body(k2, c1);
-            }
-        }
-    }
-}
 OCTA_HD inline void smp_settle(const Blk &b, int n, const unsigned short *rcnt, const unsigned short *rstart, const unsigned short *pl,
                                unsigned char *state, unsigned short *crow) {
 #if defined(__HIP_DEVICE_COMPILE__)
@@ -2264,12 +2336,8 @@
     const int n_oxy = sc->n_oxy;
     const bool single = N <= SMP_CH;
     SmpGrid G;
-    {
-        const double cell = fmax(fmax(en, es), 1.2 / SMP_GRID);
-        int nc = (int)ceil(1.2 / cell);
-        G.nc = nc < 1 ? 1 : (nc > SMP_GRID ? SMP_GRID : nc);
-        G.x0 = -0.1; G.inv = 1.0 / cell; G.endw = endw; G.pos = pos; G.live = live;
-    }
+    smp_setup(G, fmax(en, es));
+    G.endw = endw; G.pos = pos; G.live = live;
     const int nc = G.nc, nwords = (nc * nc + 2) / 2;
     const double pad = 1e-9;
     int n_pass = 0;
@@ -3539,19 +3607,56 @@
 #define OCTA_SUBPROF_T0() 0L
 #endif
 
-OCTA_HD inline void phase_satisfy_art(const Blk &b, const SimArrays &A, const SimConst &C, const IterParams &P) {
-    const double zext = C.sz;
+#if OCTA_SIM_LARGE || defined(OCTA_SIM_SATISFY_DIRECT)
+#define OCTA_SIM_SATISFY_DIRECT_FORM 1
+#else
+#define OCTA_SIM_SATISFY_DIRECT_FORM 0
+#endif
+constexpr int SAT_CH = 1024;
+constexpr int SAT_GRID = 32;
+static_assert(SAT_GRID >= 1 && SAT_GRID <= SMP_GRID, "the cell table holds SMP_GRID x SMP_GRID cells");
+constexpr size_t SAT_OFF_POS = (((size_t)SMP_GRID * SMP_GRID + 2) / 2 * 4 + 7) & ~(size_t)7, SAT_OFF_ID = SAT_OFF_POS + (size_t)SAT_CH * 24,
+                 SAT_OFF_CELL = SAT_OFF_ID + (size_t)SAT_CH * 2, SAT_OFF_RPOS = (SAT_OFF_CELL + (size_t)SAT_CH * 2 + 7) & ~(size_t)7,
+                 SAT_OFF_RID = SAT_OFF_RPOS + (size_t)SAT_CH * 24;
+static_assert(OCTA_SIM_SATISFY_DIRECT_FORM || (SAT_CH < 0xffff && SMP_GRID * SMP_GRID < 0xffff && OCAP <= 0x10000 && NCAP <= 0x10000), "slots, cells, sinks and nodes are 16-bit");
+static_assert(SAT_OFF_POS % 8 == 0 && SAT_OFF_RPOS % 8 == 0 && SAT_OFF_RID + (size_t)SAT_CH * 2 <= (size_t)SIM_USER_BYTES, "satisfied-sink tables");
+struct SatTables {
+    unsigned *endw;
+    double *pos, *rem_pos;
+    unsigned short *slot_id, *cell_of, *rem_id;
+};
+OCTA_HD inline SatTables sat_tables(const Blk &b) {
+    unsigned char *const U = b.user_of<2>();
+    SatTables T;
+    T.endw = reinterpret_cast<unsigned *>(U); T.pos = reinterpret_cast<double *>(U + SAT_OFF_POS);
+    T.slot_id = reinterpret_cast<unsigned short *>(U + SAT_OFF_ID); T.cell_of = reinterpret_cast<unsigned short *>(U + SAT_OFF_CELL);
+    T.rem_pos = reinterpret_cast<double *>(U + SAT_OFF_RPOS); T.rem_id = reinterpret_cast<unsigned short *>(U + SAT_OFF_RID);
+    return T;
+}
+#if defined(OCTA_SIM_PROF_SATISFY) && defined(__HIP_DEVICE_COMPILE__)
+#define SAT_PROF_T0() long _sat_t = (long)wall_clock64()
+#define SAT_PROF(slot) do { b.sync(); if (b.tid == 0) { long _t = (long)wall_clock64(); A.sc->kdprof[slot] += _t - _sat_t; _sat_t = _t; } } while (0)
+#else
+#define SAT_PROF_T0() do { } while (0)
+#define SAT_PROF(slot) do { } while (0)
+#endif
+
+OCTA_HD inline int *satisfy_ctl(const Blk &b) { return b.coll() + 100; }
+OCTA_HD inline unsigned char *satisfy_group_flags(const SimArrays &A) {
+    static_assert((size_t)NCAP <= (size_t)OCAP * sizeof(int), "group flags fit the nearest-node list");
+    return reinterpret_cast<unsigned char *>(A.nn);
+}
+OCTA_HD inline int satisfy_art_hits(const Blk &b, const SimArrays &A, const IterParams &P, long &t0) {
     SampleScalars *sc = A.sc;
     const int nb = sc->new_begin[0], ne = sc->new_end[0];
     const int n_new = ne - nb, n_oxy = sc->n_oxy;
-    if (n_new <= 0 || n_oxy <= 0) return;
     const double ek = P.eps_k, ek2 = ek * ek;
-    long t0 = OCTA_SUBPROF_T0();
+    int *const ctl = satisfy_ctl(b);
+    unsigned char *const xf = satisfy_group_flags(A);
+#if OCTA_SIM_SATISFY_DIRECT_FORM
+    SAT_PROF_T0();
     for (int i = b.tid; i < n_oxy; i += b.nth) A.removed[i] = 0;
-    int *ctl = b.coll() + 100;
     if (b.tid == 0) { ctl[0] = 0; ctl[1] = 0; ctl[2] = 0; }
-    unsigned char *xf = reinterpret_cast<unsigned char *>(A.nn);
-    static_assert((size_t)NCAP <= (size_t)OCAP * sizeof(int), "group flags fit the nearest-node list");
     for (int j = b.tid; j < n_new && j < NCAP; j += b.nth) xf[j] = 0;
     b.sync();
     {
@@ -3559,6 +3664,7 @@
         for (int j = b.tid; j < n_new; j += b.nth) new_ids[j] = nb + j;
         b.sync();
         Grid G = grid_build(b, A, A.npos[0], new_ids, n_new, ek);
+        SAT_PROF(0);
         for (int o = b.tid; o < n_oxy; o += b.nth) {
             const V3 p = ld3(A.oxy + 3 * o);
             grid_visit(G, p.x, p.y, ek, [&](int j, const V3 &q) {
@@ -3570,13 +3676,14 @@
             });
         }
         b.sync();
+        SAT_PROF(1);
     }
     OCTA_SUBPROF(sc, 12, t0);
     int n_pairs = ctl[0];
     if (n_pairs > PCAP) { if (b.tid == 0) atomic_or_int(&sc->err, ERR_PAIR_CAP); n_pairs = PCAP; }
     if (n_new > (1 << (32 - IDX_BITS))) { if (b.tid == 0) atomic_or_int(&sc->err, ERR_PAIR_CAP); }
     b.sync();
-    if (n_pairs == 0) return;
+    if (n_pairs == 0) return 0;
     {
         const int n_ven = sc->n_nodes[1];
         int *rem = A.tmp_int;
@@ -3598,6 +3705,7 @@
             A.hashes[o] = py_hash_tuple3(ld3(A.oxy + 3 * o));
         }
         Grid G = grid_build(b, A, A.oxy, rem, n_rem, ek);
+        SAT_PROF(2);
         constexpr int VB = 4;
         for (int j0 = b.tid; j0 < n_ven; j0 += VB * b.nth) {
             V3 qv[VB];
@@ -3613,8 +3721,112 @@
             }
         }
         b.sync();
+        SAT_PROF(3);
     }
     OCTA_SUBPROF(sc, 12, t0);
+#else
+    SAT_PROF_T0();
+    const SatTables T = sat_tables(b);
+    SmpGrid G;
+    smp_setup(G, ek, SAT_GRID);
+    G.endw = T.endw; G.pos = T.pos; G.live = nullptr;
+    const int nwords = (G.nc * G.nc + 2) / 2;
+    for (int i = b.tid; i < n_oxy; i += b.nth) A.removed[i] = 0;
+    for (int j = b.tid; j < n_new && j < NCAP; j += b.nth) xf[j] = 0;
+    if (b.tid == 0) { ctl[0] = 0; ctl[1] = 0; ctl[2] = 0; ctl[3] = 0; }
+    SAT_COUNT(0, 1); SAT_COUNT(1, n_new); SAT_COUNT(2, n_oxy);
+#if defined(OCTA_SIM_SATISFY_COUNT) && !defined(__HIP_DEVICE_COMPILE__)
+    sat_count_pass = 13;
+#endif
+    for (int base = 0; base < n_new; base += SAT_CH) {
+        const int n = n_new - base < SAT_CH ? n_new - base : SAT_CH;
+        b.sync();
+        for (int w = b.tid; w < nwords; w += b.nth) T.endw[w] = 0;
+        b.sync();
+        sat_bin(b, G, T.pos, T.slot_id, T.cell_of, A.npos[0] + 3 * (size_t)(nb + base), nullptr, base, n);
+        SAT_PROF(0);
+        sat_stream(b, G, A.oxy, n_oxy, ek,
+            [&](int o, const V3 &p, int k, const V3 &q) {
+                if (!(sqdist(p, q) <= ek2)) return false;
+                const int slot = atomic_add_int(&ctl[0], 1);
+                if (slot < PCAP) A.pairs[slot] = ((unsigned)T.slot_id[k] << IDX_BITS) | (unsigned)o;
+                return true;
+            },
+            [&](int o, const V3 &p, bool hit) {
+                if (!hit || (base && A.removed[o])) return;
+                A.removed[o] = 1;
+                const int r = atomic_add_int(&ctl[3], 1);
+                if (r < SAT_CH) { T.rem_id[r] = (unsigned short)o; st3(T.rem_pos + 3 * r, p); }
+            });
+        SAT_PROF(1);
+    }
+    b.sync();
+    OCTA_SUBPROF(sc, 12, t0);
+    int n_pairs = ctl[0];
+    const int n_rem = ctl[3];
+    SAT_COUNT(3, n_pairs); SAT_COUNT(4, n_rem);
+    if (n_pairs > PCAP) { if (b.tid == 0) atomic_or_int(&sc->err, ERR_PAIR_CAP); n_pairs = PCAP; }
+    if (n_new > (1 << (32 - IDX_BITS))) { if (b.tid == 0) atomic_or_int(&sc->err, ERR_PAIR_CAP); }
+    b.sync();
+    if (n_pairs == 0) return 0;
+    {
+        const int n_ven = sc->n_nodes[1];
+        SAT_COUNT(5, n_ven);
+#if defined(OCTA_SIM_SATISFY_COUNT) && !defined(__HIP_DEVICE_COMPILE__)
+        sat_count_pass = 14;
+#endif
+        int *rem = A.tmp_int;
+        const bool listed = n_rem <= SAT_CH;
+        if (!listed) {
+            const int chunk = (n_oxy + b.nth - 1) / b.nth;
+            const int i0 = b.tid * chunk < n_oxy ? b.tid * chunk : n_oxy, i1 = (i0 + chunk < n_oxy) ? i0 + chunk : n_oxy;
+            int local = 0;
+            for (int o = i0; o < i1; o++) local += A.removed[o] ? 1 : 0;
+            int ex;
+            blk_scan(b, local, &ex);
+            int run = ex;
+            for (int o = i0; o < i1; o++) if (A.removed[o]) rem[run++] = o;
+            SAT_COUNT(6, 1);
+        }
+        for (int base = 0; base < n_rem; base += SAT_CH) {
+            const int n = n_rem - base < SAT_CH ? n_rem - base : SAT_CH;
+            b.sync();
+            for (int w = b.tid; w < nwords; w += b.nth) T.endw[w] = 0;
+            for (int k = b.tid; k < n; k += b.nth) {
+                if (!listed) { const int o = rem[base + k]; T.rem_id[k] = (unsigned short)o; st3(T.rem_pos + 3 * k, ld3(A.oxy + 3 * (size_t)o)); }
+                const int o = T.rem_id[k];
+                A.ven_near[o] = 0;
+                A.hashes[o] = py_hash_tuple3(ld3(T.rem_pos + 3 * k));
+            }
+            b.sync();
+            sat_bin(b, G, T.pos, T.slot_id, T.cell_of, T.rem_pos, T.rem_id, 0, n);
+            SAT_PROF(2);
+            sat_stream(b, G, A.npos[1], n_ven, ek,
+                [&](int, const V3 &q, int k, const V3 &p) {
+                    if (sqrt(sqdist(q, p)) <= ek) A.ven_near[T.slot_id[k]] = 1;
+                    return false;
+                },
+                [&](int, const V3 &, bool) {});
+            SAT_PROF(3);
+        }
+        b.sync();
+    }
+    OCTA_SUBPROF(sc, 12, t0);
+#endif
+    return n_pairs;
+}
+
+OCTA_HD inline void phase_satisfy_art(const Blk &b, const SimArrays &A, const SimConst &C, const IterParams &P) {
+    const double zext = C.sz;
+    SampleScalars *sc = A.sc;
+    const int nb = sc->new_begin[0], ne = sc->new_end[0];
+    const int n_new = ne - nb, n_oxy = sc->n_oxy;
+    if (n_new <= 0 || n_oxy <= 0) return;
+    long t0 = OCTA_SUBPROF_T0();
+    int *const ctl = satisfy_ctl(b);
+    unsigned char *const xf = satisfy_group_flags(A);
+    const int n_pairs = satisfy_art_hits(b, A, P, t0);
+    if (n_pairs == 0) return;
     bool set_in_lds = false;
     int rung = 0;
     bool from_partial = false;
@@ -3967,18 +4179,20 @@
     OCTA_SUBPROF(sc, 15, t0);
 }
 
-OCTA_HD inline void phase_satisfy_ven(const Blk &b, const SimArrays &A, const IterParams &P) {
+OCTA_HD inline void satisfy_ven_flags(const Blk &b, const SimArrays &A, const IterParams &P) {
     SampleScalars *sc = A.sc;
     const int nb = sc->new_begin[1], ne = sc->new_end[1];
     const int n_new = ne - nb, n_co2 = sc->n_co2;
-    if (n_new <= 0 || n_co2 <= 0) return;
     const double ek2 = P.eps_k * P.eps_k;
     const double ek = P.eps_k;
+#if OCTA_SIM_SATISFY_DIRECT_FORM
     {
         int *new_ids = A.tmp_int;
         for (int j = b.tid; j < n_new; j += b.nth) new_ids[j] = nb + j;
         b.sync();
+        SAT_PROF_T0();
         Grid G = grid_build(b, A, A.npos[1], new_ids, n_new, ek);
+        SAT_PROF(4);
         for (int o = b.tid; o < n_co2; o += b.nth) {
             const V3 p = ld3(A.co2 + 3 * o);
             bool hit = false;
@@ -3988,7 +4202,41 @@
             A.removed[o] = hit ? 1 : 0;
         }
         b.sync();
-    }
+        SAT_PROF(5);
+    }
+#else
+    {
+        SAT_PROF_T0();
+        const SatTables T = sat_tables(b);
+        SmpGrid G;
+        smp_setup(G, ek, SAT_GRID);
+        G.endw = T.endw; G.pos = T.pos; G.live = nullptr;
+        const int nwords = (G.nc * G.nc + 2) / 2;
+        SAT_COUNT(7, 1); SAT_COUNT(8, n_new); SAT_COUNT(9, n_co2);
+#if defined(OCTA_SIM_SATISFY_COUNT) && !defined(__HIP_DEVICE_COMPILE__)
+        sat_count_pass = 15;
+#endif
+        for (int base = 0; base < n_new; base += SAT_CH) {
+            const int n = n_new - base < SAT_CH ? n_new - base : SAT_CH;
+            b.sync();
+            for (int w = b.tid; w < nwords; w += b.nth) T.endw[w] = 0;
+            b.sync();
+            sat_bin(b, G, T.pos, T.slot_id, T.cell_of, A.npos[1] + 3 * (size_t)(nb + base), nullptr, base, n);
+            SAT_PROF(4);
+            sat_stream(b, G, A.co2, n_co2, ek,
+                [&](int, const V3 &p, int, const V3 &q) { return sqdist(p, q) <= ek2; },
+                [&](int o, const V3 &, bool hit) { if (!base) A.removed[o] = hit ? 1 : 0; else if (hit) A.removed[o] = 1; });
+            SAT_PROF(5);
+        }
+        b.sync();
+    }
+#endif
+}
+OCTA_HD inline void phase_satisfy_ven(const Blk &b, const SimArrays &A, const IterParams &P) {
+    SampleScalars *sc = A.sc;
+    const int n_new = sc->new_end[1] - sc->new_begin[1], n_co2 = sc->n_co2;
+    if (n_new <= 0 || n_co2 <= 0) return;
+    satisfy_ven_flags(b, A, P);
     const bool carry = assign_memory_covers(A, 1, n_co2);
     int keep = compact_points(b, A.co2, n_co2, A.removed, A.tmp_dbl, carry ? A.nn_prev[1] : nullptr, carry ? A.nn_d2[1] : nullptr);
     if (b.tid == 0) { sc->n_co2 = keep; sc->n_cached[1] = carry ? keep : 0; }
```

Result: slower. 1382 (-9.5%).
